# JJKK1313/DiTreeOnlinePlanner

Measured on AMD Instinct MI355X. Metric: candidate tree-expansions/sec (carmaze, H=32), higher is better.
Workload: dtype f16x3; 1 GPU; cfgs/carmaze.yaml + fm_policy flow sampler (K=1), batch=1024 candidates per GPU, H=32 (4 chunks x 8 steps), boxes.csv 20x20, 1024-node tree snapshot, seeded random weights; batch_per_gpu=1024, global_batch=1024, edge_length=32, action_horizon=8, pred_horizon=64, flow_steps=1, tree_nodes=1024, parallelism=candidates sharded x1

## Files before the change

ditreeonlineplanner_amd/csrc/conv_tiles.hip:

```cpp
#include <type_traits>

#include "denoise_device.h"

static thread_local bool g_dn_dry_run = false;
void denoise_set_dry_run(bool on) { g_dn_dry_run = on; }
bool denoise_dry_run() { return g_dn_dry_run; }

template <int PREC>
__device__ __forceinline__ void gemm_epilogue(const ConvGemmParams& p, f32x16_t (&acc)[2][4], char* smem, int tm, int tn,
                                              int tid, int lane, int r5, int h, int wm, int wn,
                                              long long out_extra_bytes = 0) {

  constexpr int ET = PREC == 2 ? 1 : 0;
  float satm = 0.0f;
  const int c_l = wn * 128 + 4 * r5;
  const int n0 = tn * 256 + c_l;
  const bool n_ok = n0 < p.N;
  float bias4[4] = {0.f, 0.f, 0.f, 0.f};
  if (p.bias != nullptr && n_ok) {
    f32x4_t t = *(const f32x4_t*)(p.bias + n0);
#pragma unroll
    for (int j = 0; j < 4; ++j) bias4[j] = t[j];
  }
#pragma unroll
  for (int mb = 0; mb < 2; ++mb)
#pragma unroll
    for (int j = 0; j < 4; ++j)
#pragma unroll
      for (int i = 0; i < 16; ++i) {
        if constexpr (PREC == 2) acc[mb][j][i] = fmaf(acc[mb][j][i], p.w_scale, bias4[j]);
        else acc[mb][j][i] += bias4[j];
      }

  int blk_b[4], blk_l[4];
#pragma unroll
  for (int blk = 0; blk < 4; ++blk) {
    const int m0 = tm * 256 + wm * 64 + (blk >> 1) * 32 + (blk & 1) * 16;
    const int b = m0 / p.L;
    blk_b[blk] = b;
    blk_l[blk] = m0 - b * p.L;
  }

  if (p.mode >= MODE_GN_MISH) {
    float* s_sum = (float*)smem;
    float* s_sq = s_sum + 64;
    if (tid < 128) s_sum[tid] = 0.0f;
    const f32x4_t gam = *(const f32x4_t*)(p.gamma + n0);
    const f32x4_t bet = *(const f32x4_t*)(p.beta + n0);
    f32x4_t film_s[4], film_b[4];
    if (p.mode == MODE_GN_MISH_FILM) {
#pragma unroll
      for (int blk = 0; blk < 4; ++blk) {
        const float* fr = p.film + (long long)blk_b[blk] * p.film_ld + p.film_off + n0;
        film_s[blk] = *(const f32x4_t*)fr;
        film_b[blk] = *(const f32x4_t*)(fr + p.N);
      }
    }
    short4_t resv[2][8];
    auto fetch_res = [&](int blk, short4_t (&dst)[8]) {
#pragma unroll
      for (int i = 0; i < 8; ++i) {
        const int rofs = (i & 3) + 8 * (i >> 2) + 4 * h;
        const long long rrow = (long long)blk_b[blk] * p.res_Lp + blk_l[blk] + rofs + p.res_off;
        dst[i] = *(const short4_t*)((const char*)p.Res + (rrow * p.ldres + n0) * 2);
      }
    };
    const bool res_bf16 = (PREC != 1) && p.mode == MODE_GN_MISH_RES;
    if (res_bf16) fetch_res(0, resv[0]);
    __syncthreads();
    const int spt = 256 / p.L;
    const int gi = c_l / p.group_ch;
    const bool wide = p.group_ch >= 128;
    int slot[4];
#pragma unroll
    for (int blk = 0; blk < 4; ++blk) slot[blk] = blk_b[blk] - tm * spt;
    const float inv_cnt = 1.0f / (float)(p.group_ch * p.L);
    const bool ordered = p.L >= 128 || (p.group_ch == 256 && p.L >= 32);
    const bool adder = lane == 0 || (!wide && lane == 16);
    const int ocell = ((wm * 2 + wn) * 4 + gi) * 2;
    auto put = [&](float* cell, float (&t)[4]) {
      if (ordered) {
        if (p.L >= 64) { t[0] = (t[0] + t[1]) + (t[2] + t[3]); t[2] = 0.0f; }
        else { t[0] += t[1]; t[2] += t[3]; }
        if (adder) { cell[ocell] = t[0]; cell[ocell + 1] = t[2]; }
      } else if (adder) {
#pragma unroll
        for (int blk = 0; blk < 4; ++blk) atomicAdd(&cell[slot[blk] * 4 + gi], t[blk]);
      }
    };
    auto get = [&](const float* cell, float (&t)[4]) {
      if (!ordered) {
#pragma unroll
        for (int blk = 0; blk < 4; ++blk) t[blk] = cell[slot[blk] * 4 + gi];
        return;
      }
#pragma unroll
      for (int blk = 0; blk < 4; blk += 2) {
        const int r0 = slot[blk] * p.L;
        const int w0 = r0 >> 6, nw = p.L >= 64 ? p.L >> 6 : 1, sub = (r0 >> 5) & 1;
        float v = 0.0f;
        for (int w = w0; w < w0 + nw; ++w) {
          v += cell[((w * 2 + 0) * 4 + gi) * 2 + sub];
          v += cell[((w * 2 + 1) * 4 + gi) * 2 + sub];
        }
        t[blk] = v; t[blk + 1] = v;
      }
    };
    float mean[4], rstd[4];
    if constexpr (PREC != 1) {
      float ps[4], pq[4];
#pragma unroll
      for (int blk = 0; blk < 4; ++blk) {
        float s = 0.f, q = 0.f;
#pragma unroll
        for (int j = 0; j < 4; ++j)
#pragma unroll
          for (int i = 0; i < 8; ++i) {
            const float v = acc[blk >> 1][j][(blk & 1) * 8 + i];
            s += v;
            q = fmaf(v, v, q);
          }
        s += __shfl_xor(s, 1); q += __shfl_xor(q, 1);
        s += __shfl_xor(s, 2); q += __shfl_xor(q, 2);
        s += __shfl_xor(s, 4); q += __shfl_xor(q, 4);
        s += __shfl_xor(s, 8); q += __shfl_xor(q, 8);
        s += __shfl_xor(s, 32); q += __shfl_xor(q, 32);
        if (wide) { s += __shfl_xor(s, 16); q += __shfl_xor(q, 16); }
        ps[blk] = s; pq[blk] = q;
      }
      put(s_sum, ps);
      put(s_sq, pq);
      __syncthreads();
      get(s_sum, ps);
      get(s_sq, pq);
#pragma unroll
      for (int blk = 0; blk < 4; ++blk) {
        mean[blk] = ps[blk] * inv_cnt;
        const float var = fmaxf(pq[blk] * inv_cnt - mean[blk] * mean[blk], 0.0f);
        rstd[blk] = rsqrtf(var + p.eps);
      }
    } else {
    {
      float ps[4];
#pragma unroll
      for (int blk = 0; blk < 4; ++blk) {
        float s = 0.f;
#pragma unroll
        for (int j = 0; j < 4; ++j)
#pragma unroll
          for (int i = 0; i < 8; ++i) s += acc[blk >> 1][j][(blk & 1) * 8 + i];
        ps[blk] = s;
      }
#pragma unroll
      for (int blk = 0; blk < 4; ++blk) {
        float s = ps[blk];
        s += __shfl_xor(s, 1); s += __shfl_xor(s, 2); s += __shfl_xor(s, 4); s += __shfl_xor(s, 8);
        s += __shfl_xor(s, 32);
        if (wide) s += __shfl_xor(s, 16);
        ps[blk] = s;
      }
      put(s_sum, ps);
      __syncthreads();
      get(s_sum, ps);
#pragma unroll
      for (int blk = 0; blk < 4; ++blk) mean[blk] = ps[blk] * inv_cnt;
    }
    {
      float ps[4];
#pragma unroll
      for (int blk = 0; blk < 4; ++blk) {
        float s = 0.f;
#pragma unroll
        for (int j = 0; j < 4; ++j)
#pragma unroll
          for (int i = 0; i < 8; ++i) {
            float d = acc[blk >> 1][j][(blk & 1) * 8 + i] - mean[blk];
            s += d * d;
          }
        s += __shfl_xor(s, 1); s += __shfl_xor(s, 2); s += __shfl_xor(s, 4); s += __shfl_xor(s, 8);
        s += __shfl_xor(s, 32);
        if (wide) s += __shfl_xor(s, 16);
        ps[blk] = s;
      }
      put(s_sq, ps);
      __syncthreads();
      get(s_sq, ps);
#pragma unroll
      for (int blk = 0; blk < 4; ++blk) rstd[blk] = rsqrtf(ps[blk] * inv_cnt + p.eps);
    }

    }

#pragma unroll
    for (int blk = 0; blk < 4; ++blk) {
      if (res_bf16 && blk < 3) fetch_res(blk + 1, resv[(blk + 1) & 1]);
      f32x4_t fs = {1.f, 1.f, 1.f, 1.f}, fb = {0.f, 0.f, 0.f, 0.f};
      if (p.mode == MODE_GN_MISH_FILM) { fs = film_s[blk]; fb = film_b[blk]; }
      float ga[4], be[4];
#pragma unroll
      for (int j = 0; j < 4; ++j) { ga[j] = gam[j] * rstd[blk]; be[j] = bet[j] - mean[blk] * ga[j]; }
#pragma unroll
      for (int i = 0; i < 8; ++i) {
        const int ii = (blk & 1) * 8 + i;
        const int rofs = (i & 3) + 8 * (i >> 2) + 4 * h;
        const int b = blk_b[blk], l = blk_l[blk] + rofs;
        float v[4];
#pragma unroll
        for (int j = 0; j < 4; ++j) v[j] = mish_f<PREC == 1 ? 1 : 0>(acc[blk >> 1][j][ii] * ga[j] + be[j]) * fs[j] + fb[j];
        if (p.mode == MODE_GN_MISH_RES) {
          if constexpr (PREC != 1) {
            const short4_t rv = resv[blk & 1][i];
#pragma unroll
            for (int j = 0; j < 4; ++j) v[j] += e2f<ET>((unsigned short)rv[j]);
          } else {
            const long long rrow = (long long)b * p.res_Lp + l + p.res_off;
            const f32x4_t rv = *(const f32x4_t*)((const char*)p.Res + (rrow * p.ldres + n0) * 4);
#pragma unroll
            for (int j = 0; j < 4; ++j) v[j] += rv[j];
          }
        }
        const long long orow = (long long)b * p.out_Lp + (long long)l * p.out_stride + p.out_off;
        const long long oidx = orow * p.ldc + p.out_coff + n0;
        if constexpr (PREC == 1) {
          const f32x4_t o = {v[0], v[1], v[2], v[3]};
          *(f32x4_t*)((char*)p.Out + out_extra_bytes + oidx * 4) = o;
        } else {
          short4_t o;
          if constexpr (ET == 1) { sat_see2(satm, v[0], v[1]); sat_see2(satm, v[2], v[3]); }
#pragma unroll
          for (int j = 0; j < 4; ++j) o[j] = (short)f2e<ET>(v[j]);
          *(short4_t*)((char*)p.Out + out_extra_bytes + oidx * 2) = o;
        }
      }
    }
    if constexpr (ET == 1) sat_flush(p.sat, satm);
    return;
  }

#pragma unroll
  for (int blk = 0; blk < 4; ++blk) {
#pragma unroll
    for (int i = 0; i < 8; ++i) {
      const int ii = (blk & 1) * 8 + i;
      const int rofs = (i & 3) + 8 * (i >> 2) + 4 * h;
      const int m = tm * 256 + wm * 64 + (blk >> 1) * 32 + (blk & 1) * 16 + rofs;
      if (m >= p.M || !n_ok) continue;
      int b = blk_b[blk], l = blk_l[blk] + rofs;
      if ((p.L & 15) != 0) { b = m / p.L; l = m - b * p.L; }
      const long long orow = (long long)b * p.out_Lp + (long long)l * p.out_stride + p.out_off;
      const long long oidx = orow * p.ldc + p.out_coff + n0;
      if (p.out_f32 || PREC == 1) {
        const f32x4_t o = {acc[blk >> 1][0][ii], acc[blk >> 1][1][ii], acc[blk >> 1][2][ii], acc[blk >> 1][3][ii]};
        *(f32x4_t*)((char*)p.Out + out_extra_bytes + oidx * 4) = o;
      } else {
        short4_t o;
        if constexpr (ET == 1) { sat_see2(satm, acc[blk >> 1][0][ii], acc[blk >> 1][1][ii]); sat_see2(satm, acc[blk >> 1][2][ii], acc[blk >> 1][3][ii]); }
#pragma unroll
        for (int j = 0; j < 4; ++j) o[j] = (short)f2e<ET>(acc[blk >> 1][j][ii]);
        *(short4_t*)((char*)p.Out + out_extra_bytes + oidx * 2) = o;
      }
    }
  }
  if constexpr (ET == 1) sat_flush(p.sat, satm);
}

template <int PREC, bool C2D = false>
__global__ void __launch_bounds__(512, 2) conv_gemm_kernel(ConvGemmParams p) {
  constexpr int ES = (PREC == 1) ? 4 : 2;
  constexpr int ET = PREC == 2 ? 1 : 0;
  constexpr int EK = 128 / ES;
  constexpr int EPS = 16 / ES;
  extern __shared__ __attribute__((aligned(16))) char smem[];

  const int tid = threadIdx.x, lane = tid & 63, w = tid >> 6;
  const int r5 = lane & 31, h = lane >> 5;
  const int wm = w >> 1, wn = w & 1;
  const int ntn = (p.N + 255) >> 8;
  const int ntm = (p.M + 255) >> 8;
  const int tile = xcd_remap(blockIdx.x, ntm * ntn);
  const int tm = tile / ntn, tn = tile - tm * ntn;
  const int K = p.taps * p.Cin;
  const int kpt = p.Cin / EK;
  int nk = K / EK;
  int k_first = 0;
  long long out_extra = 0;
  if constexpr (C2D) {
    if (p.splitk > 1) {
      const int per = (nk + p.splitk - 1) / p.splitk;
      k_first = blockIdx.y * per;
      nk = min(nk - k_first, per);
      out_extra = (long long)blockIdx.y * p.slab_stride * 4;
    }
  }

  const char* Abase = (const char*)p.A;
  const char* Wbase = (const char*)p.W;
  long long aoff[4], boff[4];
#pragma unroll
  for (int q = 0; q < 4; ++q) {
    const int r = (w * 4 + q) * 8 + (lane >> 3);
    const int sw = (r >> 1) & 7;
    const int slot = (lane & 7) ^ sw;
    int m = tm * 256 + r;
    m = m < p.M ? m : p.M - 1;
    const int b = m / p.L, l = m - b * p.L;
    aoff[q] = (((long long)b * p.in_Lp + (long long)l * p.in_stride + p.in_off) * p.lda + slot * EPS) * ES;
    const int c = (r & 128) + 4 * (r & 31) + ((r >> 5) & 3);
    boff[q] = (((long long)(tn * 256 + c)) * K + slot * EPS) * ES;
  }
  const char* pa[4];
  const char* pb[4];
#pragma unroll
  for (int q = 0; q < 4; ++q) {
    pa[q] = Abase + aoff[q];
    pb[q] = Wbase + boff[q] + (long long)k_first * 128;
  }
  int kin = C2D ? (k_first % kpt) : 0;
  const long long a_tap_jump = ((long long)p.lda - (long long)p.Cin + EK) * ES;
  const char* c2_base[4];
  int c2_ih0[4], c2_iw0[4], c2_slot[4];
  int c2_tap = C2D ? (k_first / kpt) : 0;
  if constexpr (C2D) {
#pragma unroll
    for (int q = 0; q < 4; ++q) {
      const int r = (w * 4 + q) * 8 + (lane >> 3);
      int m = tm * 256 + r;
      m = m < p.M ? m : p.M - 1;
      const int b = m / p.c2_OHW, rem = m - b * p.c2_OHW;
      const int oh = rem / p.c2_OW, ow = rem - oh * p.c2_OW;
      c2_base[q] = Abase + (long long)b * p.c2_H * p.c2_W * p.Cin * ES;
      c2_ih0[q] = oh * p.c2_stride - p.c2_pad;
      c2_iw0[q] = ow * p.c2_stride - p.c2_pad;
      c2_slot[q] = ((lane & 7) ^ ((r >> 1) & 7)) * 16;
    }
  }
  auto c2_point = [&]() {
    const int kh = p.c2_kh[c2_tap], kw = p.c2_kw[c2_tap];
#pragma unroll
    for (int q = 0; q < 4; ++q) {
      const int ih = c2_ih0[q] + kh, iw = c2_iw0[q] + kw;
      const bool ok = ih >= 0 && ih < p.c2_H && iw >= 0 && iw < p.c2_W;
      const char* src = c2_base[q] + ((long long)(ih * p.c2_W + iw) * p.Cin + kin * EK) * ES;
      pa[q] = (ok ? src : (const char*)p.zero) + c2_slot[q];
    }
  };
  if constexpr (C2D) c2_point();
  auto advance = [&]() {
    ++kin;
    if constexpr (C2D) {
      if (kin == kpt) { kin = 0; ++c2_tap; }
      if (c2_tap < p.taps) c2_point();
#pragma unroll
      for (int q = 0; q < 4; ++q) pb[q] += 128;
    } else {
      long long ainc = 128;
      if (kin == kpt) { kin = 0; ainc = a_tap_jump; }
#pragma unroll
      for (int q = 0; q < 4; ++q) {
        pa[q] += ainc;
        pb[q] += 128;
      }
    }
  };
  auto stage_piece = [&](int q, char* sbase) {
    if (q < 4)
      __builtin_amdgcn_global_load_lds((const GLOBAL_AS void*)pa[q], (LDS_AS void*)(sbase + (w * 4 + q) * 1024), 16, 0, 0);
    else
      __builtin_amdgcn_global_load_lds((const GLOBAL_AS void*)pb[q - 4],
                                       (LDS_AS void*)(sbase + 32768 + (w * 4 + q - 4) * 1024), 16, 0, 0);
  };

  f32x16_t acc[2][4];
#pragma unroll
  for (int mb = 0; mb < 2; ++mb)
#pragma unroll
    for (int j = 0; j < 4; ++j)
#pragma unroll
      for (int i = 0; i < 16; ++i) acc[mb][j][i] = 0.0f;

  const int swl = (r5 >> 1) & 7;
  const int a_row_off = (wm * 64 + r5) * 128;
  const int b_row_off = 32768 + (wn * 128 + r5) * 128;

  auto kstep = [&](const char* sb, auto stage_tag, char* snext) {
    constexpr bool STAGE = decltype(stage_tag)::value;
    if constexpr (PREC != 1) {
      short8_t af[2][2], bfr[2][4];
      auto rd = [&](int ks, int slot) {
        const int ps = (((ks << 1) | h) ^ swl) << 4;
#pragma unroll
        for (int mb = 0; mb < 2; ++mb)
          af[slot][mb] = *(const short8_t*)(sb + a_row_off + mb * 4096 + ps);
#pragma unroll
        for (int j = 0; j < 4; ++j)
          bfr[slot][j] = *(const short8_t*)(sb + b_row_off + j * 4096 + ps);
      };
      if constexpr (STAGE) {
#pragma unroll
        for (int q = 0; q < 8; ++q) stage_piece(q, snext);
      }
      rd(0, 0);
#pragma unroll
      for (int ks = 0; ks < 4; ++ks) {
        if (ks < 3) rd(ks + 1, (ks + 1) & 1);
#pragma unroll
        for (int mb = 0; mb < 2; ++mb)
#pragma unroll
          for (int j = 0; j < 4; ++j)
            acc[mb][j] = mfma32<ET>(af[ks & 1][mb], bfr[ks & 1][j], acc[mb][j]);
      }
      if constexpr (STAGE) __builtin_amdgcn_sched_group_barrier(0x020, 8, 0);
      __builtin_amdgcn_sched_group_barrier(0x100, 6, 0);
#pragma unroll
      for (int ks = 0; ks < 4; ++ks) {
        if (ks < 3) __builtin_amdgcn_sched_group_barrier(0x100, 6, 0);
        __builtin_amdgcn_sched_group_barrier(0x008, 8, 0);
      }
    } else {
#pragma unroll
      for (int sl = 0; sl < 8; ++sl) {
        const int ps = (sl ^ swl) << 4;
        f32x4_t af[2], bfr[4];
#pragma unroll
        for (int mb = 0; mb < 2; ++mb) af[mb] = *(const f32x4_t*)(sb + a_row_off + mb * 4096 + ps);
#pragma unroll
        for (int j = 0; j < 4; ++j) bfr[j] = *(const f32x4_t*)(sb + b_row_off + j * 4096 + ps);
#pragma unroll
        for (int s2 = 0; s2 < 2; ++s2) {
#pragma unroll
          for (int mb = 0; mb < 2; ++mb) {
            const float a = h ? af[mb][2 * s2 + 1] : af[mb][2 * s2];
#pragma unroll
            for (int j = 0; j < 4; ++j) {
              const float bv = h ? bfr[j][2 * s2 + 1] : bfr[j][2 * s2];
              acc[mb][j] = __builtin_amdgcn_mfma_f32_32x32x2f32(a, bv, acc[mb][j], 0, 0, 0);
            }
          }
        }
        if constexpr (STAGE) stage_piece(sl, snext);
      }
    }
  };

#pragma unroll
  for (int q = 0; q < 8; ++q) stage_piece(q, smem);
  advance();
  for (int kt = 0; kt < nk - 1; ++kt) {
    asm volatile("s_waitcnt vmcnt(0)" ::: "memory");
    __syncthreads();
    kstep(smem + (kt & 1) * 65536, std::true_type{}, smem + ((kt + 1) & 1) * 65536);
    advance();
  }
  asm volatile("s_waitcnt vmcnt(0)" ::: "memory");
  __syncthreads();
  kstep(smem + ((nk - 1) & 1) * 65536, std::false_type{}, nullptr);
  __syncthreads();
  gemm_epilogue<PREC>(p, acc, smem, tm, tn, tid, lane, r5, h, wm, wn, out_extra);
}

template <int ET, bool SPLIT, bool SHORT = false>
__device__ __forceinline__ void gemm_epilogue16(const ConvGemmParams& p, f32x4_t (&acc)[4][8], char* smem, int tm, int tn,
                                                int tid, int lane, int r4, int h4, int wm, int wn) {
  const int c_l = wn * 128 + 8 * r4;
  const int n0 = tn * 256 + c_l;
  {
    f32x4_t b0 = {0.f, 0.f, 0.f, 0.f}, b1 = b0;
    if (p.bias != nullptr) { b0 = *(const f32x4_t*)(p.bias + n0); b1 = *(const f32x4_t*)(p.bias + n0 + 4); }
    if constexpr (ET == 1) {
      const float ws = p.w_scale;
#pragma unroll
      for (int mb = 0; mb < 4; ++mb)
#pragma unroll
        for (int j = 0; j < 4; ++j) { acc[mb][j] = acc[mb][j] * ws + b0[j]; acc[mb][4 + j] = acc[mb][4 + j] * ws + b1[j]; }
    } else if (p.bias != nullptr) {
#pragma unroll
      for (int mb = 0; mb < 4; ++mb)
#pragma unroll
        for (int j = 0; j < 4; ++j) { acc[mb][j] += b0[j]; acc[mb][4 + j] += b1[j]; }
    }
  }
  constexpr bool short_l = SHORT;
  const int lane_b = short_l ? (4 * h4) / p.L : 0, lane_l = -lane_b * p.L;
  int blk_b[4], blk_l[4];
#pragma unroll
  for (int mb = 0; mb < 4; ++mb) {
    const int m0 = tm * 256 + wm * 64 + mb * 16;
    const int b = m0 / p.L;
    blk_b[mb] = b;
    blk_l[mb] = m0 - b * p.L;
  }
  auto store_row = [&](char* o, const float (&v)[8]) {
    short8_t hi, lo;
    if constexpr (ET == 1) {
      sat_check_row(p.sat, v);
#pragma unroll
      for (int jj = 0; jj < 4; ++jj) {
        const f32x2_t c = {__builtin_amdgcn_fmed3f(v[2 * jj], -65504.0f, 65504.0f),
                           __builtin_amdgcn_fmed3f(v[2 * jj + 1], -65504.0f, 65504.0f)};
        const half2_t h = __builtin_convertvector(c, half2_t);
        const short2_t hs = __builtin_bit_cast(short2_t, h);
        hi[2 * jj] = hs[0]; hi[2 * jj + 1] = hs[1];
        if constexpr (SPLIT) {
          const half2_t l = __builtin_convertvector(c - __builtin_convertvector(h, f32x2_t), half2_t);
          const short2_t ls = __builtin_bit_cast(short2_t, l);
          lo[2 * jj] = ls[0]; lo[2 * jj + 1] = ls[1];
        }
      }
    } else {
#pragma unroll
      for (int j = 0; j < 8; ++j) {
        hi[j] = (short)f2bf(v[j]);
        if constexpr (SPLIT) lo[j] = (short)f2bf(v[j] - bf2f((unsigned short)hi[j]));
      }
    }
    *(short8_t*)o = hi;
    if constexpr (SPLIT) *(short8_t*)(o + p.out_plane) = lo;
  };
  auto out_ptr = [&](int mb, int esize) {
    const long long orow = (long long)(blk_b[mb] + lane_b) * p.out_Lp + (long long)(blk_l[mb] + 4 * h4 + lane_l) * p.out_stride + p.out_off;
    return (char*)p.Out + (orow * p.ldc + p.out_coff + n0) * esize;
  };
  if (p.mode < MODE_GN_MISH) {
    const int esize = p.out_f32 ? 4 : 2;
    const long long ostep = (long long)p.out_stride * p.ldc * esize;
#pragma unroll
    for (int mb = 0; mb < 4; ++mb) {
      char* ob = out_ptr(mb, esize);
#pragma unroll
      for (int i = 0; i < 4; ++i, ob += ostep) {
        float v[8];
#pragma unroll
        for (int j = 0; j < 8; ++j) v[j] = acc[mb][j][i];
        if (p.out_f32) {
          *(f32x4_t*)ob = f32x4_t{v[0], v[1], v[2], v[3]};
          *(f32x4_t*)(ob + 16) = f32x4_t{v[4], v[5], v[6], v[7]};
        } else {
          store_row(ob, v);
        }
      }
    }
    return;
  }
  const bool has_film = p.mode == MODE_GN_MISH_FILM, has_res = p.mode == MODE_GN_MISH_RES;
  const int spt = 256 / p.L;
  const int ns = spt > 16 ? spt * 4 : 64;
  float* s_sum = (float*)smem;
  float* s_sq = s_sum + ns;
  float* s_gb = s_sq + ns;
  float* s_film = s_gb + 512;
  const bool film_direct = has_film && short_l;
  const int b_last = p.M / p.L - 1;
  for (int i = tid; i < 2 * ns; i += 512) s_sum[i] = 0.0f;
  s_gb[tid] = tid < 256 ? p.gamma[tn * 256 + tid] : p.beta[tn * 256 + tid - 256];
  if (has_film && !film_direct) {
    for (int idx = tid; idx < spt * 128; idx += 512) {
      const int sm = idx >> 7, c4 = idx & 127;
      const int b = min(tm * spt + sm, b_last);
      const float* src = p.film + (long long)b * p.film_ld + p.film_off + tn * 256 + (c4 & 63) * 4 + (c4 >> 6) * p.N;
      *(f32x4_t*)(s_film + sm * 512 + c4 * 4) = *(const f32x4_t*)src;
    }
  }
  f32x4_t rh[2], rl[2];
  const long long rstep = (long long)p.ldres * 2;
  auto fetch_film = [&](int mb) {
    const float* fr = p.film + (long long)min(blk_b[mb] + lane_b, b_last) * p.film_ld + p.film_off + n0;
    rh[0] = *(const f32x4_t*)fr; rh[1] = *(const f32x4_t*)(fr + 4);
    rl[0] = *(const f32x4_t*)(fr + p.N); rl[1] = *(const f32x4_t*)(fr + p.N + 4);
  };
  if (film_direct) fetch_film(0);
  auto fetch_res = [&](int r) {
    const long long rrow = (long long)(blk_b[r >> 2] + lane_b) * p.res_Lp + blk_l[r >> 2] + 4 * h4 + lane_l + p.res_off;
    const char* rp = (const char*)p.Res + (rrow * p.ldres + n0) * 2 + (r & 3) * rstep;
    rh[r & 1] = *(const f32x4_t*)rp;
    if constexpr (SPLIT) rl[r & 1] = *(const f32x4_t*)(rp + p.res_plane);
  };
  if (has_res) { fetch_res(0); fetch_res(1); }
  __syncthreads();
  const int gi = c_l / p.group_ch;
  const bool wide = p.group_ch >= 128;
  const float inv_cnt = 1.0f / (float)(p.group_ch * p.L);
  int slot[4];
#pragma unroll
  for (int mb = 0; mb < 4; ++mb) slot[mb] = (blk_b[mb] + lane_b - tm * spt) * 4 + gi;
  const bool ordered = !short_l && (p.L >= 128 || (p.group_ch == 256 && p.L >= 32));
  const int hsame = short_l ? (p.L == 8 ? 2 : 1) : 4;
  const bool adder = (r4 == 0 || (!wide && r4 == 8)) && (h4 & (hsame - 1)) == 0;
  const int ocell = ((wm * 2 + wn) * 4 + gi) * 2;
  auto block_sums = [&](float (&s)[4], float* cell) {
#pragma unroll
    for (int mb = 0; mb < 4; ++mb) s[mb] = dpp_add<0xB1>(s[mb]);
#pragma unroll
    for (int mb = 0; mb < 4; ++mb) s[mb] = dpp_add<0x4E>(s[mb]);
#pragma unroll
    for (int mb = 0; mb < 4; ++mb) s[mb] = dpp_add<0x141>(s[mb]);
    if (wide) {
#pragma unroll
      for (int mb = 0; mb < 4; ++mb) s[mb] = dpp_add<0x140>(s[mb]);
    }
    if (hsame >= 2) {
#pragma unroll
      for (int mb = 0; mb < 4; ++mb) s[mb] += __shfl_xor(s[mb], 16);
    }
    if (hsame == 4) {
#pragma unroll
      for (int mb = 0; mb < 4; ++mb) s[mb] += __shfl_xor(s[mb], 32);
    }
    if (ordered) {
      if (p.L >= 64) { s[0] = (s[0] + s[1]) + (s[2] + s[3]); s[2] = 0.0f; }
      else { s[0] += s[1]; s[2] += s[3]; }
      if (adder) { cell[ocell] = s[0]; cell[ocell + 1] = s[2]; }
    } else if (adder) {
#pragma unroll
      for (int mb = 0; mb < 4; ++mb) atomicAdd(&cell[slot[mb]], s[mb]);
    }
  };
  auto cell_sums = [&](const float* cell, float (&t)[4]) {
    if (!ordered) {
#pragma unroll
      for (int mb = 0; mb < 4; ++mb) t[mb] = cell[slot[mb]];
      return;
    }
#pragma unroll
    for (int mb = 0; mb < 4; mb += 2) {
      const int r0 = (blk_b[mb] - tm * spt) * p.L;
      const int w0 = r0 >> 6, nw = p.L >= 64 ? p.L >> 6 : 1, sub = (r0 >> 5) & 1;
      float v = 0.0f;
      for (int w = w0; w < w0 + nw; ++w) {
        v += cell[((w * 2 + 0) * 4 + gi) * 2 + sub];
        v += cell[((w * 2 + 1) * 4 + gi) * 2 + sub];
      }
      t[mb] = v; t[mb + 1] = v;
    }
  };
  float mean_[4], rstd_[4];
  auto pair = [&](int mb, int j, int ip) { return f32x2_t{acc[mb][j][2 * ip], acc[mb][j][2 * ip + 1]}; };
  if constexpr (!SPLIT) {
    float s[4], q[4];
#pragma unroll
    for (int mb = 0; mb < 4; ++mb) {
      f32x2_t s2 = {0.f, 0.f}, q2 = {0.f, 0.f};
#pragma unroll
      for (int j = 0; j < 8; ++j)
#pragma unroll
        for (int ip = 0; ip < 2; ++ip) {
          const f32x2_t v = pair(mb, j, ip);
          s2 += v;
          q2 = __builtin_elementwise_fma(v, v, q2);
        }
      s[mb] = s2[0] + s2[1];
      q[mb] = q2[0] + q2[1];
    }
    block_sums(s, s_sum);
    block_sums(q, s_sq);
    __syncthreads();
    cell_sums(s_sum, s);
    cell_sums(s_sq, q);
#pragma unroll
    for (int mb = 0; mb < 4; ++mb) {
      mean_[mb] = s[mb] * inv_cnt;
      const float var = fmaxf(q[mb] * inv_cnt - mean_[mb] * mean_[mb], 0.0f);
      rstd_[mb] = rsqrtf(var + p.eps);
    }
  } else {
    float s[4];
#pragma unroll
    for (int mb = 0; mb < 4; ++mb) {
      f32x2_t s2 = {0.f, 0.f};
#pragma unroll
      for (int j = 0; j < 8; ++j)
#pragma unroll
        for (int ip = 0; ip < 2; ++ip) s2 += pair(mb, j, ip);
      s[mb] = s2[0] + s2[1];
    }
    block_sums(s, s_sum);
    __syncthreads();
    cell_sums(s_sum, s);
#pragma unroll
    for (int mb = 0; mb < 4; ++mb) {
      mean_[mb] = s[mb] * inv_cnt;
      f32x2_t q2 = {0.f, 0.f};
#pragma unroll
      for (int j = 0; j < 8; ++j) {
#pragma unroll
        for (int ip = 0; ip < 2; ++ip) {
          const f32x2_t d = pair(mb, j, ip) - mean_[mb];
          q2 = __builtin_elementwise_fma(d, d, q2);
        }
        if (j & 1) __builtin_amdgcn_sched_barrier(0);
      }
      s[mb] = q2[0] + q2[1];
    }
    block_sums(s, s_sq);
    __syncthreads();
    cell_sums(s_sq, s);
#pragma unroll
    for (int mb = 0; mb < 4; ++mb) rstd_[mb] = rsqrtf(s[mb] * inv_cnt + p.eps);
  }
  const long long ostep = (long long)p.out_stride * p.ldc * 2;
#pragma unroll
  for (int mb = 0; mb < 4; ++mb) {
    float mean = mean_[mb];
    const float rstd = rstd_[mb];
    if constexpr (SPLIT) asm volatile("" : "+v"(mean));
    float ga[8], be[8], fs[8], fb[8];
    {
      const f32x4_t gam0 = *(const f32x4_t*)(s_gb + c_l), gam1 = *(const f32x4_t*)(s_gb + c_l + 4);
      const f32x4_t bet0 = *(const f32x4_t*)(s_gb + 256 + c_l), bet1 = *(const f32x4_t*)(s_gb + 256 + c_l + 4);
#pragma unroll
      for (int j = 0; j < 4; ++j) {
        ga[j] = gam0[j] * rstd; ga[4 + j] = gam1[j] * rstd;
        if constexpr (SPLIT) { be[j] = bet0[j]; be[4 + j] = bet1[j]; }
        else { be[j] = bet0[j] - mean * ga[j]; be[4 + j] = bet1[j] - mean * ga[4 + j]; }
      }
    }
    if (film_direct) {
#pragma unroll
      for (int j = 0; j < 4; ++j) { fs[j] = rh[0][j]; fs[4 + j] = rh[1][j]; fb[j] = rl[0][j]; fb[4 + j] = rl[1][j]; }
      if (mb + 1 < 4) fetch_film(mb + 1);
    } else if (has_film) {
      const float* fr = s_film + (blk_b[mb] - tm * spt) * 512 + c_l;
      const f32x4_t f0 = *(const f32x4_t*)fr, f1 = *(const f32x4_t*)(fr + 4);
      const f32x4_t f2 = *(const f32x4_t*)(fr + 256), f3 = *(const f32x4_t*)(fr + 260);
#pragma unroll
      for (int j = 0; j < 4; ++j) { fs[j] = f0[j]; fs[4 + j] = f1[j]; fb[j] = f2[j]; fb[4 + j] = f3[j]; }
    }
    char* ob = out_ptr(mb, 2);
#pragma unroll
    for (int ip = 0; ip < 2; ++ip, ob += 2 * ostep) {
      const int r = mb * 4 + 2 * ip;
      f32x2_t v[8];
      if (has_res) {
        const short8_t h0 = __builtin_bit_cast(short8_t, rh[0]), h1 = __builtin_bit_cast(short8_t, rh[1]);
#pragma unroll
        for (int j = 0; j < 8; ++j) v[j] = f32x2_t{e2f<ET>((unsigned short)h0[j]), e2f<ET>((unsigned short)h1[j])};
        if constexpr (SPLIT) {
          const short8_t l0 = __builtin_bit_cast(short8_t, rl[0]), l1 = __builtin_bit_cast(short8_t, rl[1]);
#pragma unroll
          for (int j = 0; j < 8; ++j) v[j] += f32x2_t{e2f<ET>((unsigned short)l0[j]), e2f<ET>((unsigned short)l1[j])};
        }
        if (r + 2 < 16) { fetch_res(r + 2); fetch_res(r + 3); }
      } else {
#pragma unroll
        for (int j = 0; j < 8; ++j) v[j] = f32x2_t{0.f, 0.f};
      }
#pragma unroll
      for (int j = 0; j < 8; ++j) {
        f32x2_t x = pair(mb, j, ip);
        if constexpr (SPLIT) x = (x - mean) * ga[j] + be[j];
        else x = x * ga[j] + be[j];
        x = mish2<SPLIT ? 2 : 0>(x);
        v[j] += x;
      }
      if (has_film) {
#pragma unroll
        for (int j = 0; j < 8; ++j) v[j] = v[j] * fs[j] + fb[j];
      }
      float row[8];
#pragma unroll
      for (int j = 0; j < 8; ++j) row[j] = v[j][0];
      store_row(ob, row);
#pragma unroll
      for (int j = 0; j < 8; ++j) row[j] = v[j][1];
      store_row(ob + ostep, row);
      __builtin_amdgcn_sched_barrier(0);
    }
  }
}

template <int ET>
__device__ __forceinline__ void mm16_snake(f32x4_t (&acc)[4][8], const short8_t (&a)[4], const short8_t (&b)[4], int half) {
#pragma unroll
  for (int mb = 0; mb < 4; ++mb)
#pragma unroll
    for (int jj = 0; jj < 4; ++jj) {
      const int j = (mb & 1) ? 3 - jj : jj;
      acc[mb][half * 4 + j] = mfma16<ET>(a[mb], b[j], acc[mb][half * 4 + j]);
    }
}

#ifdef HALO16_STAMP
__device__ unsigned long long g_halo_stamp[8];
extern "C" int ditree_debug_halo_stamp(unsigned long long* out) {
  return (int)hipMemcpyFromSymbol(out, HIP_SYMBOL(g_halo_stamp), sizeof(g_halo_stamp));
}
__device__ unsigned int g_x3_phase[8][32];
extern "C" int ditree_debug_x3_phase(unsigned int* out) {
  return (int)hipMemcpyFromSymbol(out, HIP_SYMBOL(g_x3_phase), sizeof(g_x3_phase));
}
#define X3_STAMP_MAX 65536
__device__ unsigned long long g_x3_stamp[X3_STAMP_MAX][6];
__device__ unsigned int g_x3_count;
extern "C" int ditree_debug_x3_stamp(unsigned long long* out, unsigned int* count, int reset) {
  int rc = (int)hipMemcpyFromSymbol(count, HIP_SYMBOL(g_x3_count), 4);
  if (rc == 0 && out != nullptr) rc = (int)hipMemcpyFromSymbol(out, HIP_SYMBOL(g_x3_stamp), sizeof(unsigned long long) * 6 * X3_STAMP_MAX);
  if (rc == 0 && reset) { unsigned int z = 0; rc = (int)hipMemcpyToSymbol(HIP_SYMBOL(g_x3_count), &z, 4); }
  return rc;
}
#endif
template <int ET>
__global__ void __launch_bounds__(512, 2) conv3_halo16_kernel(ConvGemmParams p) {
  extern __shared__ __attribute__((aligned(16))) char smem[];
  constexpr int A_BUF = 40960, W_BUF = 32768, W_BASE = 2 * A_BUF;
  const int tid = threadIdx.x, lane = tid & 63;
  const int w = __builtin_amdgcn_readfirstlane(tid >> 6);
  const int r4 = lane & 15, h4 = lane >> 4;
  const int wm = w >> 1, wn = w & 1;
  const int ntn = (p.N + 255) >> 8;
  const int ntm = (p.M + 255) >> 8;
  const int tile = xcd_remap_strips(blockIdx.x, ntm, ntn, p.xcd_strips);
  const int tm = tile / ntn, tn = tile - tm * ntn;
  const int L = p.L, Lp = p.in_Lp, S = 256 / L;
  const int a_rows = S * Lp;
  const int nc = p.Cin >> 6;
  const long long K = 3LL * p.Cin;

  unsigned pa0, pa4, pb;
  const char* const a_base = (const char*)p.A + ((long long)tm * S * Lp + p.in_off) * p.lda * 2;
  const char* const w_base = (const char*)p.W + ((long long)tn * 256) * K * 2;
  const __amdgpu_buffer_rsrc_t a_rsrc = __builtin_amdgcn_make_buffer_rsrc((void*)a_base, 0, 0x7fffffff, 0x00020000);
  const __amdgpu_buffer_rsrc_t w_rsrc = __builtin_amdgcn_make_buffer_rsrc((void*)w_base, 0, 0x7fffffff, 0x00020000);
  {
    const int r = w * 8 + (lane >> 3);
    const int slot = (lane & 7) ^ (r & 7);
    pa0 = (unsigned)((r * p.lda + slot * 8) * 2);
    const int r4r = r + 256;
    const int rs = r4r < a_rows ? r4r : a_rows - 1;
    pa4 = (unsigned)((rs * p.lda + slot * 8) * 2);
  }
  const int a_piece = 64 * p.lda * 2;
  long long wq[4];
  {
    const int lr = lane >> 3;
    const int slot = (lane & 7) ^ lr;
    pb = (unsigned)(((long long)(8 * lr) * K + slot * 8) * 2);
#pragma unroll
    for (int q = 0; q < 4; ++q) {
      const int r0 = (w * 4 + q) * 8;
      const int cu = (r0 & 128) + 8 * (r0 & 8) + ((r0 >> 4) & 7);
      wq[q] = (long long)cu * K * 2;
    }
  }
  const int w_tap = p.Cin * 2;
  auto issue_a = [&](int c, int i) {
    __builtin_amdgcn_raw_ptr_buffer_load_lds(a_rsrc, (LDS_AS void*)(smem + (c & 1) * A_BUF + (w + 8 * i) * 1024), 16,
                                             i < 4 ? pa0 : pa4, c * 128 + (i < 4 ? i * a_piece : 0), 0, 0);
  };
  auto issue_w = [&](int c, int t, int q) {
    __builtin_amdgcn_raw_ptr_buffer_load_lds(w_rsrc, (LDS_AS void*)(smem + W_BASE + ((c + t) & 1) * W_BUF + (w * 4 + q) * 1024),
                                             16, pb, (int)wq[q] + c * 128 + t * w_tap, 0, 0);
  };

  int lrow0;
  {
    const int ml = wm * 64 + r4;
    const int sb = ml / L;
    lrow0 = sb * Lp + (ml - sb * L);
  }
  int lstep[4];
#pragma unroll
  for (int mb = 0; mb < 4; ++mb) lstep[mb] = 16 * mb + 2 * (((wm * 64 + 16 * mb) / L) - ((wm * 64) / L));
  const int swl = r4 & 7;
  const int b_row_off = (wn * 128 + r4) * 128;

  f32x4_t acc[4][8];
#pragma unroll
  for (int mb = 0; mb < 4; ++mb)
#pragma unroll
    for (int j = 0; j < 8; ++j) acc[mb][j] = f32x4_t{0.f, 0.f, 0.f, 0.f};

  short8_t af[2][4], bq[2][4];
  auto rdA = [&](int set, int c, int t, int ks) {
    const char* ab = smem + (c & 1) * A_BUF;
#pragma unroll
    for (int mb = 0; mb < 4; ++mb) {
      const int row = lrow0 + lstep[mb] + t;
      const int ps = (((ks << 2) | h4) ^ (row & 7)) << 4;
      af[set][mb] = *(const short8_t*)(ab + row * 128 + ps);
    }
  };
  auto rdB = [&](int set, int c, int t, int ks, int half) {
    const char* wb = smem + W_BASE + ((c + t) & 1) * W_BUF + b_row_off + half * 8192;
    const int psb = (((ks << 2) | h4) ^ swl) << 4;
#pragma unroll
    for (int jj = 0; jj < 4; ++jj) bq[set][jj] = *(const short8_t*)(wb + jj * 2048 + psb);
  };
  auto mm = [&](int aset, int bset, int half, int mb, int jj) {
    acc[mb][half * 4 + jj] = mfma16<ET>(af[aset][mb], bq[bset][jj], acc[mb][half * 4 + jj]);
  };
  auto mm16 = [&](int aset, int bset, int half) { mm16_snake<ET>(acc, af[aset], bq[bset], half); };

  auto step = [&](auto tT, auto tNext, auto tIW, auto tIA, auto tVM, int c) {
    constexpr int T = decltype(tT)::value;
    constexpr bool HAS_NEXT = decltype(tNext)::value, ISSUE_W = decltype(tIW)::value, ISSUE_A = decltype(tIA)::value;
    constexpr int VM = decltype(tVM)::value;
    constexpr int NV = ISSUE_W ? 4 : 0;
    asm volatile("" : "+v"(lrow0));
    __builtin_amdgcn_s_setprio(2);
    rdB(1, c, T, 0, 1);
    mm16(0, 0, 0);
    __builtin_amdgcn_sched_group_barrier(0x100, 4, 0);
    __builtin_amdgcn_sched_group_barrier(0x008, 16, 0);
    __builtin_amdgcn_sched_barrier(0);
    __builtin_amdgcn_s_setprio(1);
    rdA(1, c, T, 1);
    rdB(0, c, T, 1, 0);
    mm16(0, 1, 1);
    __builtin_amdgcn_sched_group_barrier(0x100, 8, 0);
    __builtin_amdgcn_sched_group_barrier(0x008, 16, 0);
    __builtin_amdgcn_sched_barrier(0);
    __builtin_amdgcn_s_setprio(0);
    rdB(1, c, T, 1, 1);
    mm16(1, 0, 0);
    if constexpr (ISSUE_A && T != 2) {
      if constexpr (T == 0) { issue_a(c + 1, 0); issue_a(c + 1, 1); issue_a(c + 1, 2); }
      else { issue_a(c + 1, 3); issue_a(c + 1, 4); }
      __builtin_amdgcn_sched_group_barrier(0x100, 4, 0);
      __builtin_amdgcn_sched_group_barrier(0x008, 4, 0);
      __builtin_amdgcn_sched_group_barrier(0x020, 1, 0);
      __builtin_amdgcn_sched_group_barrier(0x008, 4, 0);
      __builtin_amdgcn_sched_group_barrier(0x020, 1, 0);
      __builtin_amdgcn_sched_group_barrier(0x008, 4, 0);
      if constexpr (T == 0) __builtin_amdgcn_sched_group_barrier(0x020, 1, 0);
      __builtin_amdgcn_sched_group_barrier(0x008, 4, 0);
    } else {
      __builtin_amdgcn_sched_group_barrier(0x100, 4, 0);
      __builtin_amdgcn_sched_group_barrier(0x008, 16, 0);
    }
    __builtin_amdgcn_sched_barrier(0);
    if constexpr (HAS_NEXT) {
      if constexpr (VM == 0) asm volatile("s_waitcnt vmcnt(0) lgkmcnt(0)" ::: "memory");
      else if constexpr (VM == 3) asm volatile("s_waitcnt vmcnt(3) lgkmcnt(0)" ::: "memory");
      else asm volatile("s_waitcnt vmcnt(2) lgkmcnt(0)" ::: "memory");
      __builtin_amdgcn_s_barrier();
      __builtin_amdgcn_s_setprio(3);
      constexpr int T1 = (T + 1) % 3;
      rdA(0, c + (T + 1) / 3, T1, 0);
      rdB(0, c + (T + 1) / 3, T1, 0, 0);
    }
    constexpr int T2 = (T + 2) % 3;
    const int c2 = c + (T + 2) / 3;
#pragma unroll
    for (int mb = 0; mb < 4; ++mb)
#pragma unroll
      for (int jj = 0; jj < 4; ++jj) {
        mm(1, 1, 1, mb, (mb & 1) ? 3 - jj : jj);
        const int i = mb * 4 + jj;
        const int d = (i & 1) ? -1 : (i >> 1);
        if constexpr (ISSUE_W) { if (d >= 0 && d < 4) issue_w(c2, T2, d); }
      }
    if constexpr (HAS_NEXT) __builtin_amdgcn_sched_group_barrier(0x100, 8, 1);
#pragma unroll
    for (int i = 0; i < 16; ++i) {
      __builtin_amdgcn_sched_group_barrier(0x008, 1, 1);
      if (!(i & 1) && (i >> 1) < NV) __builtin_amdgcn_sched_group_barrier(0x020, 1, 1);
    }
    __builtin_amdgcn_sched_barrier(0);
  };
  using I0 = std::integral_constant<int, 0>;
  using I1 = std::integral_constant<int, 1>;
  using I2 = std::integral_constant<int, 2>;
  using I3 = std::integral_constant<int, 3>;
  using Tt = std::true_type;
  using Ff = std::false_type;

#pragma unroll
  for (int i = 0; i < 5; ++i) issue_a(0, i);
#pragma unroll
  for (int q = 0; q < 4; ++q) issue_w(0, 0, q);
  asm volatile("s_waitcnt vmcnt(0)" ::: "memory");
  __builtin_amdgcn_s_barrier();
#pragma unroll
  for (int q = 0; q < 4; ++q) issue_w(0, 1, q);
  rdA(0, 0, 0, 0);
  rdB(0, 0, 0, 0, 0);

#ifdef HALO16_STAMP
  const unsigned long long st0 = __builtin_amdgcn_s_memtime(), rt0 = __builtin_amdgcn_s_memrealtime();
#endif
  for (int c = 0; c < nc - 2; ++c) {
    step(I0{}, Tt{}, Tt{}, Tt{}, I3{}, c);
    step(I1{}, Tt{}, Tt{}, Tt{}, I2{}, c);
    step(I2{}, Tt{}, Tt{}, Tt{}, I0{}, c);
  }
#ifdef HALO16_STAMP
  if (blockIdx.x == 100 && tid == 0 && nc >= 32) {
    g_halo_stamp[0] = __builtin_amdgcn_s_memtime() - st0;
    g_halo_stamp[1] = __builtin_amdgcn_s_memrealtime() - rt0;
    g_halo_stamp[2] = (unsigned long long)(nc - 2) * 3;
  }
#endif
  {
    const int c = nc - 2;
    step(I0{}, Tt{}, Tt{}, Tt{}, I0{}, c);
    step(I1{}, Tt{}, Tt{}, Tt{}, I0{}, c);
    step(I2{}, Tt{}, Tt{}, Ff{}, I0{}, c);
  }
  {
    const int c = nc - 1;
    step(I0{}, Tt{}, Tt{}, Ff{}, I0{}, c);
    step(I1{}, Tt{}, Ff{}, Ff{}, I0{}, c);
    step(I2{}, Ff{}, Ff{}, Ff{}, I0{}, c);
  }
  __builtin_amdgcn_s_setprio(0);
  __syncthreads();
  gemm_epilogue16<ET, false>(p, acc, smem, tm, tn, tid, lane, r4, h4, wm, wn);
}

template <int ET, bool SHORT = false, bool SPLITK = false, int NP = 5>
__global__ void __launch_bounds__(512, 2) conv3_halo16x3_kernel(ConvGemmParams p) {
  extern __shared__ __attribute__((aligned(16))) char smem[];
  static_assert(NP == 5 || NP == 6, "five or six activation pieces");
  constexpr int A_BUF = NP * 8192, W_BUF = 32768, W_BASE = 2 * A_BUF;
  const int tid = threadIdx.x, lane = tid & 63;
  const int w = __builtin_amdgcn_readfirstlane(tid >> 6);
  const int r4 = lane & 15, h4 = lane >> 4;
  const int wm = w >> 1, wn = w & 1;
  const int ntn = (p.N + 255) >> 8;
  const int ntm = (p.M + 255) >> 8;
  const int tile = xcd_remap_strips(blockIdx.x, ntm, ntn, p.xcd_strips);
  const int tm = tile / ntn, tn = tile - tm * ntn;
  const int L = p.L, Lp = p.in_Lp, S = 256 / L;
  const int a_rows = S * Lp;
  const int nv_all = p.Cin >> 5;
  const int v_lo = SPLITK ? (int)blockIdx.y * (nv_all / p.splitk) : 0;
  const int nv = SPLITK ? v_lo + nv_all / p.splitk : nv_all;
  const long long w_row = p.w_row;
  const int w_step = p.w_step;
  const unsigned a_plane = (unsigned)p.a_plane, w_plane = (unsigned)p.w_plane;

  unsigned pa0, pa4, pa5 = 0, pb;
  const char* const a_base = (const char*)p.A + ((long long)tm * S * Lp + p.in_off) * p.lda * 2;
  const char* const w_base = (const char*)p.W + ((long long)tn * 256) * w_row;
  const __amdgpu_buffer_rsrc_t a_rsrc = __builtin_amdgcn_make_buffer_rsrc((void*)a_base, 0, 0x7fffffff, 0x00020000);
  const __amdgpu_buffer_rsrc_t w_rsrc = __builtin_amdgcn_make_buffer_rsrc((void*)w_base, 0, 0x7fffffff, 0x00020000);
  {
    const int r = w * 8 + (lane >> 3);
    const int slot = (lane & 7) ^ (r & 7);
    const unsigned po = (slot & 4) ? a_plane : 0u;
    pa0 = (unsigned)((r * p.lda + (slot & 3) * 8) * 2) + po;
    const int r4r = r + 256;
    const int rs = r4r < a_rows ? r4r : a_rows - 1;
    pa4 = (unsigned)((rs * p.lda + (slot & 3) * 8) * 2) + po;
    if constexpr (NP == 6) {
      const int r5r = r + 320;
      const int rs5 = r5r < a_rows ? r5r : a_rows - 1;
      pa5 = (unsigned)((rs5 * p.lda + (slot & 3) * 8) * 2) + po;
    }
  }
  const int a_piece = 64 * p.lda * 2;
  long long wq[4];
  {
    const int lr = lane >> 3;
    const int slot = (lane & 7) ^ lr;
    pb = (unsigned)((long long)(8 * lr) * w_row + (slot & 3) * 16) + ((slot & 4) ? w_plane : 0u);
#pragma unroll
    for (int q = 0; q < 4; ++q) {
      const int r0 = (w * 4 + q) * 8;
      const int cu = (r0 & 128) + 8 * (r0 & 8) + ((r0 >> 4) & 7);
      wq[q] = (long long)cu * w_row;
    }
  }
  const int w_tap = (p.Cin >> 5) * w_step;
  auto issue_a = [&](int v, int i) {
    __builtin_amdgcn_raw_ptr_buffer_load_lds(a_rsrc, (LDS_AS void*)(smem + (v & 1) * A_BUF + (w + 8 * i) * 1024), 16,
                                             i < 4 ? pa0 : (i == 4 ? pa4 : pa5), v * 64 + (i < 4 ? i * a_piece : 0), 0, 0);
  };
  auto issue_w = [&](int v, int t, int q) {
    __builtin_amdgcn_raw_ptr_buffer_load_lds(w_rsrc, (LDS_AS void*)(smem + W_BASE + ((v + t) & 1) * W_BUF + (w * 4 + q) * 1024),
                                             16, pb, (int)wq[q] + v * w_step + t * w_tap, 0, 0);
  };

  int lrow0;
  {
    const int ml = wm * 64 + r4;
    const int sb = ml / L;
    lrow0 = sb * Lp + (ml - sb * L);
  }
  int lstep[4];
#pragma unroll
  for (int mb = 0; mb < 4; ++mb) lstep[mb] = 16 * mb + 2 * (((wm * 64 + 16 * mb) / L) - ((wm * 64) / L));
  const int swl = r4 & 7;
  const int b_row_off = (wn * 128 + r4) * 128;

  f32x4_t acc[4][8];
#pragma unroll
  for (int mb = 0; mb < 4; ++mb)
#pragma unroll
    for (int j = 0; j < 8; ++j) acc[mb][j] = f32x4_t{0.f, 0.f, 0.f, 0.f};

  short8_t af[2][4], bq[2][4];
  auto rdA = [&](int set, int v, int t, int pl) {
    const char* ab = smem + (v & 1) * A_BUF;
#pragma unroll
    for (int mb = 0; mb < 4; ++mb) {
      const int row = lrow0 + lstep[mb] + t;
      const int ps = (((pl << 2) | h4) ^ (row & 7)) << 4;
      af[set][mb] = *(const short8_t*)(ab + row * 128 + ps);
    }
  };
  auto rdB = [&](int set, int v, int t, int pl, int half) {
    const char* wb = smem + W_BASE + ((v + t) & 1) * W_BUF + b_row_off + half * 8192;
    const int psb = (((pl << 2) | h4) ^ swl) << 4;
#pragma unroll
    for (int jj = 0; jj < 4; ++jj) bq[set][jj] = *(const short8_t*)(wb + jj * 2048 + psb);
  };
  auto mm = [&](int aset, int bset, int half, int mb, int jj) {
    acc[mb][half * 4 + jj] = mfma16<ET>(af[aset][mb], bq[bset][jj], acc[mb][half * 4 + jj]);
  };
  auto mm16 = [&](int aset, int bset, int half) { mm16_snake<ET>(acc, af[aset], bq[bset], half); };

#ifdef X3_PHASE_STAMP
  unsigned pst[24];
#define PSTAMP(k) do { pst[T * 8 + (k)] = (unsigned)__builtin_amdgcn_s_memtime(); __builtin_amdgcn_sched_barrier(0); } while (0)
#else
#define PSTAMP(k) do { } while (0)
#endif
  auto step = [&](auto tT, auto tNext, auto tIW, auto tIA, auto tVM, int v) {
    constexpr int T = decltype(tT)::value;
    constexpr bool HAS_NEXT = decltype(tNext)::value, ISSUE_W = decltype(tIW)::value, ISSUE_A = decltype(tIA)::value;
    constexpr int VM = decltype(tVM)::value;
    asm volatile("" : "+v"(lrow0));
    PSTAMP(0);
    __builtin_amdgcn_s_setprio(2);
    rdB(1, v, T, 1, 1);
    mm16(0, 0, 0);
    __builtin_amdgcn_sched_group_barrier(0x100, 4, 0);
    __builtin_amdgcn_sched_group_barrier(0x008, 16, 0);
    __builtin_amdgcn_sched_barrier(0);
    PSTAMP(1);
    rdB(0, v, T, 0, 0);
    rdA(1, v, T, 1);
    mm16(0, 1, 1);
    __builtin_amdgcn_sched_group_barrier(0x100, 8, 0);
    __builtin_amdgcn_sched_group_barrier(0x008, 16, 0);
    __builtin_amdgcn_sched_barrier(0);
    PSTAMP(2);
    __builtin_amdgcn_s_setprio(1);
    rdB(1, v, T, 0, 1);
    mm16(0, 0, 0);
    __builtin_amdgcn_sched_group_barrier(0x100, 4, 0);
    __builtin_amdgcn_sched_group_barrier(0x008, 16, 0);
    __builtin_amdgcn_sched_barrier(0);
    PSTAMP(3);
    mm16(1, 0, 0);
    if constexpr (ISSUE_A && T != 2) {
      if constexpr (T == 0) { issue_a(v + 1, 0); issue_a(v + 1, 1); issue_a(v + 1, 2); }
      else { issue_a(v + 1, 3); issue_a(v + 1, 4); if constexpr (NP == 6) issue_a(v + 1, 5); }
      __builtin_amdgcn_sched_group_barrier(0x008, 4, 2);
      __builtin_amdgcn_sched_group_barrier(0x020, 1, 2);
      __builtin_amdgcn_sched_group_barrier(0x008, 4, 2);
      __builtin_amdgcn_sched_group_barrier(0x020, 1, 2);
      __builtin_amdgcn_sched_group_barrier(0x008, 4, 2);
      if constexpr (T == 0 || NP == 6) __builtin_amdgcn_sched_group_barrier(0x020, 1, 2);
      __builtin_amdgcn_sched_group_barrier(0x008, 4, 2);
    }
    __builtin_amdgcn_sched_barrier(0);
    PSTAMP(4);
    __builtin_amdgcn_s_setprio(0);
    mm16(0, 1, 1);
    __builtin_amdgcn_sched_barrier(0);
    PSTAMP(5);
    if constexpr (HAS_NEXT) {
      if constexpr (VM == 0) asm volatile("s_waitcnt vmcnt(0) lgkmcnt(0)" ::: "memory");
      else if constexpr (VM == 3) asm volatile("s_waitcnt vmcnt(3) lgkmcnt(0)" ::: "memory");
      else asm volatile("s_waitcnt vmcnt(2) lgkmcnt(0)" ::: "memory");
      __builtin_amdgcn_s_barrier();
      __builtin_amdgcn_s_setprio(3);
      PSTAMP(6);
      constexpr int T1 = (T + 1) % 3;
      rdA(0, v + (T + 1) / 3, T1, 0);
      rdB(0, v + (T + 1) / 3, T1, 1, 0);
    }
    constexpr int T2 = (T + 2) % 3;
    const int v2 = v + (T + 2) / 3;
#pragma unroll
    for (int mb = 0; mb < 4; ++mb)
#pragma unroll
      for (int jj = 0; jj < 4; ++jj) {
        mm(1, 1, 1, mb, (mb & 1) ? 3 - jj : jj);
        const int i = mb * 4 + jj;
        const int d = (i & 1) ? -1 : (i >> 1);
        if constexpr (ISSUE_W) { if (d >= 0 && d < 4) issue_w(v2, T2, d); }
      }
    if constexpr (HAS_NEXT) __builtin_amdgcn_sched_group_barrier(0x100, 8, 1);
    constexpr int NV = ISSUE_W ? 4 : 0;
#pragma unroll
    for (int i = 0; i < 16; ++i) {
      __builtin_amdgcn_sched_group_barrier(0x008, 1, 1);
      if (!(i & 1) && (i >> 1) < NV) __builtin_amdgcn_sched_group_barrier(0x020, 1, 1);
    }
    __builtin_amdgcn_sched_barrier(0);
    PSTAMP(7);
  };
#undef PSTAMP
  using I0 = std::integral_constant<int, 0>;
  using I1 = std::integral_constant<int, 1>;
  using I2 = std::integral_constant<int, 2>;
  using I3 = std::integral_constant<int, 3>;
  using Tt = std::true_type;
  using Ff = std::false_type;

#ifdef HALO16_STAMP
  const unsigned long long xs0 = __builtin_amdgcn_s_memrealtime();
#endif
#pragma unroll
  for (int i = 0; i < NP; ++i) issue_a(v_lo, i);
#pragma unroll
  for (int q = 0; q < 4; ++q) issue_w(v_lo, 0, q);
  asm volatile("s_waitcnt vmcnt(0)" ::: "memory");
  __builtin_amdgcn_s_barrier();
#pragma unroll
  for (int q = 0; q < 4; ++q) issue_w(v_lo, 1, q);
  rdA(0, v_lo, 0, 0);
  rdB(0, v_lo, 0, 1, 0);
#ifdef HALO16_STAMP
  const unsigned long long xs1 = __builtin_amdgcn_s_memrealtime();
#endif

  using IT1 = std::integral_constant<int, NP == 6 ? 3 : 2>;
  for (int v = v_lo; v < nv - 2; ++v) {
    step(I0{}, Tt{}, Tt{}, Tt{}, I3{}, v);
    step(I1{}, Tt{}, Tt{}, Tt{}, IT1{}, v);
    step(I2{}, Tt{}, Tt{}, Tt{}, I0{}, v);
  }
#ifdef X3_PHASE_STAMP
  if (blockIdx.x == 100 && lane == 0 && nv == 64) {
#pragma unroll
    for (int k = 0; k < 24; ++k) g_x3_phase[w][k] = pst[k];
    g_x3_phase[w][24] = (unsigned)nv;
  }
#endif
  {
    const int v = nv - 2;
    step(I0{}, Tt{}, Tt{}, Tt{}, I0{}, v);
    step(I1{}, Tt{}, Tt{}, Tt{}, I0{}, v);
    step(I2{}, Tt{}, Tt{}, Ff{}, I0{}, v);
  }
  {
    const int v = nv - 1;
    step(I0{}, Tt{}, Tt{}, Ff{}, I0{}, v);
    step(I1{}, Tt{}, Ff{}, Ff{}, I0{}, v);
    step(I2{}, Ff{}, Ff{}, Ff{}, I0{}, v);
  }
  __builtin_amdgcn_s_setprio(0);
  __syncthreads();
#ifdef HALO16_STAMP
  const unsigned long long xs2 = __builtin_amdgcn_s_memrealtime();
#endif
  if constexpr (SPLITK) {
    const int ntiles = ntm * ntn;
    float* mine = p.sk_ws + ((size_t)blockIdx.y * ntiles + tile) * 65536;
#pragma unroll
    for (int mb = 0; mb < 4; ++mb)
#pragma unroll
      for (int j = 0; j < 8; ++j) *(f32x4_t*)(mine + ((mb * 8 + j) * 512 + tid) * 4) = acc[mb][j];
    __threadfence();
    __syncthreads();
    int* s_last = (int*)smem;
    if (tid == 0) *s_last = atomicAdd(p.sk_cnt + tile, 1) == p.splitk - 1;
    __syncthreads();
    const bool last = *s_last != 0;
    __syncthreads();
    if (!last) return;
    __threadfence();
#pragma unroll
    for (int mb = 0; mb < 4; ++mb)
#pragma unroll
      for (int j = 0; j < 8; ++j) acc[mb][j] = f32x4_t{0.f, 0.f, 0.f, 0.f};
    for (int sp = 0; sp < p.splitk; ++sp) {
      const float* sl = p.sk_ws + ((size_t)sp * ntiles + tile) * 65536;
#pragma unroll
      for (int mb = 0; mb < 4; ++mb)
#pragma unroll
        for (int j = 0; j < 8; ++j) acc[mb][j] += *(const f32x4_t*)(sl + ((mb * 8 + j) * 512 + tid) * 4);
    }
    if (tid == 0) p.sk_cnt[tile] = 0;
  }
  gemm_epilogue16<ET, true, SHORT>(p, acc, smem, tm, tn, tid, lane, r4, h4, wm, wn);
#ifdef HALO16_STAMP
  __syncthreads();
  if (tid == 0) {
    const unsigned long long xs3 = __builtin_amdgcn_s_memrealtime();
    const unsigned int k = atomicAdd(&g_x3_count, 1u);
    if (k < X3_STAMP_MAX) {
      g_x3_stamp[k][0] = xs0; g_x3_stamp[k][1] = xs1; g_x3_stamp[k][2] = xs2; g_x3_stamp[k][3] = xs3;
      g_x3_stamp[k][4] = ((unsigned long long)nv << 32) | blockIdx.x;
      g_x3_stamp[k][5] = ((unsigned long long)__builtin_amdgcn_s_getreg((31 << 11) | 20) << 32) |
                         (unsigned int)__builtin_amdgcn_s_getreg((31 << 11) | 4);
    }
  }
#endif
}

template <int ET, bool SPLIT>
__global__ void __launch_bounds__(256) conv2d_small_kernel(ConvGemmParams p) {
  extern __shared__ __attribute__((aligned(16))) char smem[];
  constexpr int STAGE = 16384;
  constexpr int CK = SPLIT ? 32 : 64;
  const int tid = threadIdx.x, lane = tid & 63;
  const int w = __builtin_amdgcn_readfirstlane(tid >> 6);
  const int r5 = lane & 31, h = lane >> 5;
  const int wm = w >> 1, wn = w & 1;
  const int ntn = p.N >> 6;
  const int tm = blockIdx.x / ntn, tn = blockIdx.x - tm * ntn;
  const int kpt = p.Cin / CK;
  const long long K = (long long)p.taps * p.Cin;
  int k0 = 0, nk = p.taps * kpt;
  long long out_extra = 0;
  if (p.splitk > 1) {
    const int per = (nk + p.splitk - 1) / p.splitk;
    k0 = blockIdx.y * per;
    nk = min(nk - k0, per);
    out_extra = (long long)blockIdx.y * p.slab_stride;
  }

  const char* a_base[2];
  int ih0[2], iw0[2];
  const char* w_src[2];
  int slot_b[2];
  long long plane_a[2];
#pragma unroll
  for (int q = 0; q < 2; ++q) {
    const int r = (2 * w + q) * 8 + (lane >> 3);
    const int slot = (lane & 7) ^ ((r >> 1) & 7);
    slot_b[q] = SPLIT ? (slot & 3) * 16 : slot * 16;
    plane_a[q] = (SPLIT && (slot & 4)) ? p.a_plane : 0;
    const long long plane_w = (SPLIT && (slot & 4)) ? p.w_plane : 0;
    int m = tm * 64 + r;
    m = m < p.M ? m : p.M - 1;
    const int b = m / p.c2_OHW, rem = m - b * p.c2_OHW;
    const int oh = rem / p.c2_OW, ow = rem - oh * p.c2_OW;
    a_base[q] = (const char*)p.A + (long long)b * p.c2_H * p.c2_W * p.Cin * 2;
    ih0[q] = oh * p.c2_stride - p.c2_pad;
    iw0[q] = ow * p.c2_stride - p.c2_pad;
    w_src[q] = (const char*)p.W + (long long)(tn * 64 + r) * (SPLIT ? (long long)p.w_row : K * 2) + slot_b[q] + plane_w;
  }
  auto issue = [&](int kl) {
    const int k = k0 + kl;
    const int tap = k / kpt, kin = k - tap * kpt;
    const int kh = p.c2_kh[tap], kw = p.c2_kw[tap];
    char* st = smem + (kl % 3) * STAGE;
#pragma unroll
    for (int q = 0; q < 2; ++q) {
      const int ih = ih0[q] + kh, iw = iw0[q] + kw;
      const bool ok = ih >= 0 && ih < p.c2_H && iw >= 0 && iw < p.c2_W;
      const char* src = ok ? a_base[q] + ((long long)(ih * p.c2_W + iw) * p.Cin + kin * CK) * 2 + plane_a[q] : (const char*)p.zero;
      __builtin_amdgcn_global_load_lds((const GLOBAL_AS void*)(src + slot_b[q]), (LDS_AS void*)(st + (2 * w + q) * 1024), 16, 0, 0);
    }
#pragma unroll
    for (int q = 0; q < 2; ++q)
      __builtin_amdgcn_global_load_lds((const GLOBAL_AS void*)(w_src[q] + (long long)k * (SPLIT ? p.w_step : 128)),
                                       (LDS_AS void*)(st + 8192 + (2 * w + q) * 1024), 16, 0, 0);
  };

  f32x16_t acc;
#pragma unroll
  for (int i = 0; i < 16; ++i) acc[i] = 0.0f;
  const int a_row = wm * 32 + r5, b_row = wn * 32 + r5;
  const int a_off = a_row * 128, b_off = 8192 + b_row * 128;
  const int sa = (a_row >> 1) & 7, sb = (b_row >> 1) & 7;

  issue(0);
  if (nk > 1) issue(1);
  for (int k = 0; k < nk; ++k) {
    if (k + 1 < nk) asm volatile("s_waitcnt vmcnt(4)" ::: "memory");
    else asm volatile("s_waitcnt vmcnt(0)" ::: "memory");
    __builtin_amdgcn_s_barrier();
    if (k + 2 < nk) issue(k + 2);
    const char* st = smem + (k % 3) * STAGE;
    if constexpr (SPLIT) {
      short8_t af[4], bf[4];
#pragma unroll
      for (int ks = 0; ks < 4; ++ks) {
        af[ks] = *(const short8_t*)(st + a_off + ((((ks << 1) | h) ^ sa) << 4));
        bf[ks] = *(const short8_t*)(st + b_off + ((((ks << 1) | h) ^ sb) << 4));
      }
#pragma unroll
      for (int kk = 0; kk < 2; ++kk) acc = mfma32<ET>(af[kk], bf[kk + 2], acc);
#pragma unroll
      for (int kk = 0; kk < 2; ++kk) acc = mfma32<ET>(af[kk], bf[kk], acc);
#pragma unroll
      for (int kk = 0; kk < 2; ++kk) acc = mfma32<ET>(af[kk + 2], bf[kk], acc);
    } else {
#pragma unroll
      for (int ks = 0; ks < 4; ++ks) {
        const short8_t af = *(const short8_t*)(st + a_off + ((((ks << 1) | h) ^ sa) << 4));
        const short8_t bf = *(const short8_t*)(st + b_off + ((((ks << 1) | h) ^ sb) << 4));
        acc = mfma32<ET>(af, bf, acc);
      }
    }
    asm volatile("s_waitcnt lgkmcnt(0)" ::: "memory");
  }

  const int n = tn * 64 + wn * 32 + r5;
  float bias = (p.bias != nullptr && k0 == 0) ? p.bias[n] : 0.0f;
#pragma unroll
  for (int i = 0; i < 16; ++i) {
    const int m = tm * 64 + wm * 32 + (i & 3) + 8 * (i >> 2) + 4 * h;
    if (m < p.M) ((float*)p.Out)[out_extra + (long long)m * p.ldc + p.out_coff + n] = (ET == 1 ? acc[i] * p.w_scale : acc[i]) + bias;
  }
}

template <int ET, bool SPLIT, bool SHORT = false>
__global__ void __launch_bounds__(512, 2) gemm16_kernel(ConvGemmParams p) {
  extern __shared__ __attribute__((aligned(16))) char smem[];
  constexpr int BUF = 32768, W_BASE = 2 * BUF;
  const int tid = threadIdx.x, lane = tid & 63;
  const int w = __builtin_amdgcn_readfirstlane(tid >> 6);
  const int r4 = lane & 15, h4 = lane >> 4;
  const int wm = w >> 1, wn = w & 1;
  const int ntn = p.N >> 8, ntm = p.M >> 8;
  const int tile = xcd_remap_strips(blockIdx.x, ntm, ntn, p.xcd_strips);
  const int tm = tile / ntn, tn = tile - tm * ntn;
  constexpr int KB = SPLIT ? 64 : 128;
  const int nc = SPLIT ? (p.Cin >> 5) : (p.Cin >> 6), nk = p.taps * nc;
  const unsigned a_plane = (unsigned)p.a_plane, w_plane = (unsigned)p.w_plane;
  const long long K = (long long)p.taps * p.Cin;

  long long a_tile0;
  {
    const int m0 = tm * 256;
    const int b0 = m0 / p.L, l0 = m0 - b0 * p.L;
    a_tile0 = (((long long)b0 * p.in_Lp + (long long)l0 * p.in_stride + p.in_off) * p.lda) * 2;
  }
  const __amdgpu_buffer_rsrc_t a_rsrc =
      __builtin_amdgcn_make_buffer_rsrc((void*)((const char*)p.A + a_tile0), 0, 0x7fffffff, 0x00020000);
  const long long w_row = SPLIT ? (long long)p.w_row : K * 2;
  const int w_step = SPLIT ? p.w_step : 128;
  const __amdgpu_buffer_rsrc_t w_rsrc =
      __builtin_amdgcn_make_buffer_rsrc((void*)((const char*)p.W + ((long long)tn * 256) * w_row), 0, 0x7fffffff, 0x00020000);
  unsigned pae, pao, pbe, pbo;
  int aq[4], wq[4];
  {
    const int lr = lane >> 3;
    const int slot0 = (lane & 7) ^ (lr >> 1), slot1 = slot0 ^ 4;
    const int lrb = lr / p.L, lro = lrb * p.in_Lp + (lr - lrb * p.L) * p.in_stride;
    if constexpr (SPLIT) {
      pae = (unsigned)((lro * p.lda + (slot0 & 3) * 8) * 2) + ((slot0 & 4) ? a_plane : 0u);
      pao = (unsigned)((lro * p.lda + (slot1 & 3) * 8) * 2) + ((slot1 & 4) ? a_plane : 0u);
      pbe = (unsigned)((long long)(8 * lr) * w_row + (slot0 & 3) * 16) + ((slot0 & 4) ? w_plane : 0u);
      pbo = (unsigned)((long long)(8 * lr) * w_row + (slot1 & 3) * 16) + ((slot1 & 4) ? w_plane : 0u);
    } else {
      pae = (unsigned)((lro * p.lda + slot0 * 8) * 2);
      pao = (unsigned)((lro * p.lda + slot1 * 8) * 2);
      pbe = (unsigned)(((long long)(8 * lr) * K + slot0 * 8) * 2);
      pbo = (unsigned)(((long long)(8 * lr) * K + slot1 * 8) * 2);
    }
#pragma unroll
    for (int q = 0; q < 4; ++q) {
      const int r0 = (w * 4 + q) * 8;
      const int m = tm * 256 + r0;
      const int b = m / p.L, l = m - b * p.L;
      aq[q] = (int)((((long long)b * p.in_Lp + (long long)l * p.in_stride + p.in_off) * p.lda) * 2 - a_tile0);
      const int cu = (r0 & 128) + 8 * (r0 & 8) + ((r0 >> 4) & 7);
      wq[q] = (int)((long long)cu * w_row);
    }
  }
  const int tap_bytes = p.lda * 2;
  auto src_off = [&](int k, int& ao, int& wo) {
    const int t = k / nc, c = k - t * nc;
    ao = t * tap_bytes + c * KB;
    wo = k * w_step;
  };
  auto issue = [&](int kv) {
    int ao, wo;
    src_off(kv, ao, wo);
    char* ab = smem + (kv & 1) * BUF;
    char* wb = smem + W_BASE + (kv & 1) * BUF;
#pragma unroll
    for (int q = 0; q < 4; ++q)
      __builtin_amdgcn_raw_ptr_buffer_load_lds(a_rsrc, (LDS_AS void*)(ab + (w * 4 + q) * 1024), 16, (q & 1) ? pao : pae,
                                               aq[q] + ao, 0, 0);
#pragma unroll
    for (int q = 0; q < 4; ++q)
      __builtin_amdgcn_raw_ptr_buffer_load_lds(w_rsrc, (LDS_AS void*)(wb + (w * 4 + q) * 1024), 16, (q & 1) ? pbo : pbe,
                                               wq[q] + wo, 0, 0);
  };

  auto issue_wq = [&](int kv, int q) {
    int ao, wo;
    src_off(kv, ao, wo);
    __builtin_amdgcn_raw_ptr_buffer_load_lds(w_rsrc, (LDS_AS void*)(smem + W_BASE + (kv & 1) * BUF + (w * 4 + q) * 1024), 16,
                                             (q & 1) ? pbo : pbe, wq[q] + wo, 0, 0);
  };
  const int a_row = wm * 64 + r4;
  const int swa = (a_row >> 1) & 7;
  const int a_off = a_row * 128, b_off = (wn * 128 + r4) * 128;
  const int swb = (r4 >> 1) & 7;

  f32x4_t acc[4][8];
#pragma unroll
  for (int mb = 0; mb < 4; ++mb)
#pragma unroll
    for (int j = 0; j < 8; ++j) acc[mb][j] = f32x4_t{0.f, 0.f, 0.f, 0.f};
  short8_t af[2][4], bq[2][4];
  auto rdA = [&](int set, int k, int ks) {
    const char* ab = smem + (k & 1) * BUF + a_off + ((((ks << 2) | h4) ^ swa) << 4);
#pragma unroll
    for (int mb = 0; mb < 4; ++mb) af[set][mb] = *(const short8_t*)(ab + mb * 2048);
  };
  auto rdB = [&](int set, int k, int ks, int half) {
    const char* wb = smem + W_BASE + (k & 1) * BUF + b_off + half * 8192 + ((((ks << 2) | h4) ^ swb) << 4);
#pragma unroll
    for (int jj = 0; jj < 4; ++jj) bq[set][jj] = *(const short8_t*)(wb + jj * 2048);
  };
  auto mm = [&](int aset, int bset, int half, int mb, int jj) {
    acc[mb][half * 4 + jj] = mfma16<ET>(af[aset][mb], bq[bset][jj], acc[mb][half * 4 + jj]);
  };
  auto mm16 = [&](int aset, int bset, int half) {
#pragma unroll
    for (int mb = 0; mb < 4; ++mb)
#pragma unroll
      for (int jj = 0; jj < 4; ++jj) mm(aset, bset, half, mb, (mb & 1) ? 3 - jj : jj);
  };
  auto step = [&](auto tNext, auto tIssue, int k) {
    constexpr bool HAS_NEXT = decltype(tNext)::value, ISSUE = decltype(tIssue)::value;
    if constexpr (SPLIT) {
      rdB(1, k, 1, 1);
      mm16(0, 0, 0);
      if constexpr (HAS_NEXT) {
        issue_wq(k + 1, 0); issue_wq(k + 1, 1);
        __builtin_amdgcn_sched_group_barrier(0x100, 4, 0);
        __builtin_amdgcn_sched_group_barrier(0x008, 4, 0);
        __builtin_amdgcn_sched_group_barrier(0x020, 1, 0);
        __builtin_amdgcn_sched_group_barrier(0x008, 4, 0);
        __builtin_amdgcn_sched_group_barrier(0x020, 1, 0);
        __builtin_amdgcn_sched_group_barrier(0x008, 8, 0);
      } else
      {
      __builtin_amdgcn_sched_group_barrier(0x100, 4, 0);
      __builtin_amdgcn_sched_group_barrier(0x008, 16, 0);
      }
      __builtin_amdgcn_sched_barrier(0);
      rdB(0, k, 0, 0);
      rdA(1, k, 1);
      mm16(0, 1, 1);
      if constexpr (HAS_NEXT) {
        issue_wq(k + 1, 2); issue_wq(k + 1, 3);
        __builtin_amdgcn_sched_group_barrier(0x100, 8, 0);
        __builtin_amdgcn_sched_group_barrier(0x008, 4, 0);
        __builtin_amdgcn_sched_group_barrier(0x020, 1, 0);
        __builtin_amdgcn_sched_group_barrier(0x008, 4, 0);
        __builtin_amdgcn_sched_group_barrier(0x020, 1, 0);
        __builtin_amdgcn_sched_group_barrier(0x008, 8, 0);
      } else
      {
      __builtin_amdgcn_sched_group_barrier(0x100, 8, 0);
      __builtin_amdgcn_sched_group_barrier(0x008, 16, 0);
      }
      __builtin_amdgcn_sched_barrier(0);
      rdB(1, k, 0, 1);
      mm16(0, 0, 0);
      __builtin_amdgcn_sched_group_barrier(0x100, 4, 0);
      __builtin_amdgcn_sched_group_barrier(0x008, 16, 0);
      __builtin_amdgcn_sched_barrier(0);
      mm16(1, 0, 0);
      __builtin_amdgcn_sched_barrier(0);
      mm16(0, 1, 1);
      __builtin_amdgcn_sched_barrier(0);
    } else {
      rdB(1, k, 0, 1);
      mm16(0, 0, 0);
      __builtin_amdgcn_sched_group_barrier(0x100, 4, 0);
      __builtin_amdgcn_sched_group_barrier(0x008, 16, 0);
      __builtin_amdgcn_sched_barrier(0);
      rdA(1, k, 1);
      rdB(0, k, 1, 0);
      mm16(0, 1, 1);
      __builtin_amdgcn_sched_group_barrier(0x100, 8, 0);
      __builtin_amdgcn_sched_group_barrier(0x008, 16, 0);
      __builtin_amdgcn_sched_barrier(0);
      rdB(1, k, 1, 1);
      mm16(1, 0, 0);
      __builtin_amdgcn_sched_group_barrier(0x100, 4, 0);
      __builtin_amdgcn_sched_group_barrier(0x008, 16, 0);
      __builtin_amdgcn_sched_barrier(0);
    }
    int ao2 = 0, wo2 = 0;
    if constexpr (ISSUE) src_off(k + 2, ao2, wo2);
    if constexpr (HAS_NEXT) {
      asm volatile("s_waitcnt vmcnt(0) lgkmcnt(0)" ::: "memory");
      __builtin_amdgcn_s_barrier();
      rdA(0, k + 1, 0);
      rdB(0, k + 1, SPLIT ? 1 : 0, 0);
    }
#pragma unroll
    for (int mb = 0; mb < 4; ++mb)
#pragma unroll
      for (int jj = 0; jj < 4; ++jj) {
        mm(1, 1, 1, mb, (mb & 1) ? 3 - jj : jj);
        if constexpr (ISSUE) {
          const int m = mb * 4 + jj, i = (m & 1) ? -1 : (m >> 1);
          if (i >= 0 && i < 4)
            __builtin_amdgcn_raw_ptr_buffer_load_lds(a_rsrc, (LDS_AS void*)(smem + (k & 1) * BUF + (w * 4 + i) * 1024), 16,
                                                     (i & 1) ? pao : pae, aq[i] + ao2, 0, 0);
          else if (!SPLIT && i >= 4 && i < 8)
            __builtin_amdgcn_raw_ptr_buffer_load_lds(w_rsrc, (LDS_AS void*)(smem + W_BASE + (k & 1) * BUF + (w * 4 + i - 4) * 1024),
                                                     16, ((i - 4) & 1) ? pbo : pbe, wq[i - 4] + wo2, 0, 0);
        }
      }
    if constexpr (HAS_NEXT) __builtin_amdgcn_sched_group_barrier(0x100, 8, 1);
#pragma unroll
    for (int i = 0; i < 16; ++i) {
      __builtin_amdgcn_sched_group_barrier(0x008, 1, 1);
      if (ISSUE && !(i & 1) && (!SPLIT || i < 8)) __builtin_amdgcn_sched_group_barrier(0x020, 1, 1);
    }
    __builtin_amdgcn_sched_barrier(0);
  };
  using Tt = std::true_type;
  using Ff = std::false_type;

  issue(0);
  asm volatile("s_waitcnt vmcnt(0)" ::: "memory");
  __builtin_amdgcn_s_barrier();
  if (nk > 1) {
    if constexpr (SPLIT) {
      int ao, wo;
      src_off(1, ao, wo);
#pragma unroll
      for (int q = 0; q < 4; ++q)
        __builtin_amdgcn_raw_ptr_buffer_load_lds(a_rsrc, (LDS_AS void*)(smem + BUF + (w * 4 + q) * 1024), 16, (q & 1) ? pao : pae,
                                                 aq[q] + ao, 0, 0);
    } else {
      issue(1);
    }
  }
  rdA(0, 0, 0);
  rdB(0, 0, SPLIT ? 1 : 0, 0);
  for (int k = 0; k < nk - 2; ++k) step(Tt{}, Tt{}, k);
  if (nk >= 2) step(Tt{}, Ff{}, nk - 2);
  step(Ff{}, Ff{}, nk - 1);
  __syncthreads();
  gemm_epilogue16<ET, SPLIT, SHORT>(p, acc, smem, tm, tn, tid, lane, r4, h4, wm, wn);
}
enum { TILE_HALO, TILE_GEMM16, TILE_C2D_SMALL, TILE_GENERIC };
enum { TV_SPLIT = 1,
       TV_SHORT = 2,
       TV_SPLITK = 4,
       TV_NP6 = 8,
       TV_C2D = 16 };
struct TileVariant {
  void (*kernel)(ConvGemmParams);
  unsigned lds_bytes;
  unsigned block;
  int family, st;
  unsigned flags;
  int kind;
};
static const TileVariant k_tiles[] = {
    {conv3_halo16_kernel<0>, 147456, 512, TILE_HALO, ST_BF16, 0, 0},
    {conv3_halo16_kernel<1>, 147456, 512, TILE_HALO, ST_F16, 0, 0},
    {conv3_halo16x3_kernel<0>, 147456, 512, TILE_HALO, ST_BF16, TV_SPLIT, 0},
    {conv3_halo16x3_kernel<1>, 147456, 512, TILE_HALO, ST_F16, TV_SPLIT, 0},
    {conv3_halo16x3_kernel<0, true>, 147456, 512, TILE_HALO, ST_BF16, TV_SPLIT | TV_SHORT, 0},
    {conv3_halo16x3_kernel<1, true>, 147456, 512, TILE_HALO, ST_F16, TV_SPLIT | TV_SHORT, 0},
    {conv3_halo16x3_kernel<0, false, true>, 147456, 512, TILE_HALO, ST_BF16, TV_SPLIT | TV_SPLITK, 0},
    {conv3_halo16x3_kernel<1, false, true>, 147456, 512, TILE_HALO, ST_F16, TV_SPLIT | TV_SPLITK, 0},
    {conv3_halo16x3_kernel<0, true, true>, 147456, 512, TILE_HALO, ST_BF16, TV_SPLIT | TV_SHORT | TV_SPLITK, 0},
    {conv3_halo16x3_kernel<1, true, true>, 147456, 512, TILE_HALO, ST_F16, TV_SPLIT | TV_SHORT | TV_SPLITK, 0},
    {conv3_halo16x3_kernel<0, true, false, 6>, 163840, 512, TILE_HALO, ST_BF16, TV_SPLIT | TV_SHORT | TV_NP6, 0},
    {conv3_halo16x3_kernel<1, true, false, 6>, 163840, 512, TILE_HALO, ST_F16, TV_SPLIT | TV_SHORT | TV_NP6, 0},
    {gemm16_kernel<0, false>, 131072, 512, TILE_GEMM16, ST_BF16, 0, 1},
    {gemm16_kernel<1, false>, 131072, 512, TILE_GEMM16, ST_F16, 0, 1},
    {gemm16_kernel<0, true>, 131072, 512, TILE_GEMM16, ST_BF16, TV_SPLIT, 1},
    {gemm16_kernel<1, true>, 131072, 512, TILE_GEMM16, ST_F16, TV_SPLIT, 1},
    {gemm16_kernel<0, false, true>, 131072, 512, TILE_GEMM16, ST_BF16, TV_SHORT, 1},
    {gemm16_kernel<1, false, true>, 131072, 512, TILE_GEMM16, ST_F16, TV_SHORT, 1},
    {gemm16_kernel<0, true, true>, 131072, 512, TILE_GEMM16, ST_BF16, TV_SPLIT | TV_SHORT, 1},
    {gemm16_kernel<1, true, true>, 131072, 512, TILE_GEMM16, ST_F16, TV_SPLIT | TV_SHORT, 1},
    {conv2d_small_kernel<0, false>, 3 * 16384, 256, TILE_C2D_SMALL, ST_BF16, TV_C2D, 2},
    {conv2d_small_kernel<1, false>, 3 * 16384, 256, TILE_C2D_SMALL, ST_F16, TV_C2D, 2},
    {conv2d_small_kernel<0, true>, 3 * 16384, 256, TILE_C2D_SMALL, ST_BF16, TV_C2D | TV_SPLIT, 2},
    {conv2d_small_kernel<1, true>, 3 * 16384, 256, TILE_C2D_SMALL, ST_F16, TV_C2D | TV_SPLIT, 2},
    {conv_gemm_kernel<0, false>, 131072, 512, TILE_GENERIC, ST_BF16, 0, 1},
    {conv_gemm_kernel<1, false>, 131072, 512, TILE_GENERIC, ST_F32, 0, 1},
    {conv_gemm_kernel<2, false>, 131072, 512, TILE_GENERIC, ST_F16, 0, 1},
    {conv_gemm_kernel<0, true>, 131072, 512, TILE_GENERIC, ST_BF16, TV_C2D, 2},
    {conv_gemm_kernel<1, true>, 131072, 512, TILE_GENERIC, ST_F32, TV_C2D, 2},
    {conv_gemm_kernel<2, true>, 131072, 512, TILE_GENERIC, ST_F16, TV_C2D, 2},
};
static const TileVariant* find_tile(int family, int st, unsigned flags) {
  for (const TileVariant& v : k_tiles)
    if (v.family == family && v.st == st && v.flags == flags) return &v;
  return nullptr;
}

static const TileVariant* pick_tile(const ConvGemmParams& p, int fmt) {
  const int st = fmt_st(fmt);
  const bool split = fmt_split(fmt);
  const unsigned fsplit = split ? TV_SPLIT : 0;
  const bool tile16 = st != ST_F32 && !p.c2d && (p.M & 255) == 0 && (p.N & 255) == 0 && (p.Cin & 63) == 0;
  const bool l_ok = p.L >= 16 || (p.L == 8 && split) || (p.L == 4 && split && p.splitk <= 1);
  if (tile16 && p.taps == 3 && p.in_stride == 1 && p.in_Lp == p.L + 2 && (256 % p.L) == 0 && l_ok && p.Cin >= 192) {
    if (!split) return find_tile(TILE_HALO, st, 0);
    const unsigned fshort = p.L <= 8 ? TV_SHORT : 0;
    if (p.splitk > 1) return find_tile(TILE_HALO, st, TV_SPLIT | fshort | TV_SPLITK);
    return find_tile(TILE_HALO, st, TV_SPLIT | fshort | (p.L == 4 ? TV_NP6 : 0));
  }
  const bool short_l = p.L == 8 || p.L == 4;
  if (tile16 && (!p.out_f32 || p.mode == MODE_BIAS) && p.taps >= 1 && p.taps <= 3 && ((p.L & 15) == 0 || short_l) && p.M > 0 &&
      (p.mode == MODE_BIAS || (256 % p.L) == 0))
    return find_tile(TILE_GEMM16, st, fsplit | ((p.L & 15) != 0 ? TV_SHORT : 0));
  if (p.c2d && conv2d_small_eligible(fmt) && (p.N & 63) == 0 && (p.Cin & 63) == 0 && p.out_f32 && p.mode == MODE_BIAS)
    return find_tile(TILE_C2D_SMALL, st, TV_C2D | fsplit);
  if (split) return nullptr;
  return find_tile(TILE_GENERIC, st, p.c2d ? TV_C2D : 0);
}
bool conv2d_small_eligible(int fmt) { return fmt_st(fmt) != ST_F32; }
int conv_gemm_kind(const ConvGemmParams& p, int fmt) {
  const TileVariant* v = pick_tile(p, fmt);
  return v != nullptr ? v->kind : (p.c2d ? 2 : 1);
}
bool conv_gemm_supported(const ConvGemmParams& p, int fmt) { return pick_tile(p, fmt) != nullptr; }

static void ensure_lds_attrs() {
  static bool done[64] = {};
  int dev = 0;
  hipGetDevice(&dev);
  if (dev < 0 || dev >= 64 || done[dev]) return;
  done[dev] = true;
  for (const TileVariant& v : k_tiles)
    if (v.lds_bytes > 65536) hipFuncSetAttribute((const void*)v.kernel, hipFuncAttributeMaxDynamicSharedMemorySize, (int)v.lds_bytes);
}

void launch_conv_gemm(const ConvGemmParams& p, int fmt, hipStream_t s) {
  ensure_lds_attrs();
  const TileVariant* v = pick_tile(p, fmt);
  if (v != nullptr && (v->flags & TV_SPLITK) &&
      (p.sk_ws == nullptr || p.sk_cnt == nullptr || ((p.Cin >> 5) % p.splitk) != 0 || (p.Cin >> 5) / p.splitk < 2))
    throw std::runtime_error("conv_gemm: split-K of the halo kernel needs its workspace and splitk | Cin / 32, >= 2 chunks each");
  if ((v == nullptr || v->family == TILE_GENERIC) && p.mode >= MODE_GN_MISH && (p.L & 15) != 0)
    throw std::runtime_error("conv_gemm: a fused GroupNorm epilogue at L = 8 / 4 exists on the gemm16 tile only (whole 256-row tiles)");
  if (v == nullptr) throw std::runtime_error("conv_gemm: a split GEMM of this shape fits no tile (conv_gemm_supported is the contract)");
  dim3 grid(((p.M + 255) >> 8) * ((p.N + 255) >> 8));
  if (v->family == TILE_C2D_SMALL) grid.x = ((p.M + 63) >> 6) * (p.N >> 6);
  if (v->flags & (TV_SPLITK | TV_C2D)) grid.y = p.splitk > 1 ? p.splitk : 1;
  DN_LAUNCH(v->kernel, grid, dim3(v->block), v->lds_bytes, s, p);
}
```

Before: 19320 candidate expansions/s.

## Specialize halo conv kernels on sequence length to precompute LDS fragment addresses

Adds L-specialized variants of the halo-tiled conv3 kernels for L = 16, 32 and 64. In these variants the per-fragment LDS row steps are compile-time constants, so the swizzled base addresses can be precomputed once and the inner loop issues ds_reads with immediate offsets. The main loop is also unrolled by two chunks so the double-buffer parity is a compile-time constant, which removes VALU address arithmetic between the MFMAs. The tile picker routes matching shapes to the new variants. The cost is more template instantiations and extra live address registers, which could raise VGPR pressure or perturb the hand-tuned schedule; a probe script for counting the loop's instruction mix is included.

```diff
diff --git a/ditreeonlineplanner_amd/csrc/conv_tiles.hip b/ditreeonlineplanner_amd/csrc/conv_tiles.hip
--- a/ditreeonlineplanner_amd/csrc/conv_tiles.hip
+++ b/ditreeonlineplanner_amd/csrc/conv_tiles.hip
@@ -777,6 +777,24 @@
       acc[mb][half * 4 + j] = mfma16<ET>(a[mb], b[j], acc[mb][half * 4 + j]);
     }
 }
+
+template <int LM>
+__device__ __forceinline__ constexpr int halo_frag_step(int mb) {
+  return LM == 16 ? 18 * mb : LM == 32 ? 16 * mb + 2 * (mb >> 1) : 16 * mb;
+}
+template <int LM>
+__device__ __forceinline__ constexpr unsigned halo_frag_keys() {
+  unsigned m = 0;
+  for (int mb = 0; mb < 4; ++mb)
+    for (int t = 0; t < 3; ++t) m |= 1u << ((halo_frag_step<LM>(mb) + t) & 7);
+  return m;
+}
+template <int LM>
+__device__ __forceinline__ void halo_frag_bases(unsigned (&abase)[8], unsigned lds0, int lrow0, int h4) {
+#pragma unroll
+  for (int k = 0; k < 8; ++k) abase[k] = LM != 0 ? lds0 + (unsigned)(lrow0 * 128 + ((h4 ^ ((lrow0 + k) & 7)) << 4)) : 0u;
+}
+__device__ __forceinline__ short8_t halo_frag_read(unsigned addr) { return *(const LDS_AS short8_t*)(size_t)addr; }
 
 #ifdef HALO16_STAMP
 __device__ unsigned long long g_halo_stamp[8];
@@ -797,9 +815,10 @@
   return rc;
 }
 #endif
-template <int ET>
-__global__ void __launch_bounds__(512, 2) conv3_halo16_kernel(ConvGemmParams p) {
-  extern __shared__ __attribute__((aligned(16))) char smem[];
+template <int ET, int LM>
+__device__ __forceinline__ void conv3_halo16_body(const ConvGemmParams& p) {
+  extern __shared__ __attribute__((aligned(128))) char smem_halo[];
+  static_assert(LM == 0 || LM == 16 || LM == 32 || LM == 64, "L at run time, or L = 16, 32, 64 (halo_frag_step)");
   constexpr int A_BUF = 40960, W_BUF = 32768, W_BASE = 2 * A_BUF;
   const int tid = threadIdx.x, lane = tid & 63;
   const int w = __builtin_amdgcn_readfirstlane(tid >> 6);
@@ -841,12 +860,12 @@
     }
   }
   const int w_tap = p.Cin * 2;
-  auto issue_a = [&](int c, int i) {
-    __builtin_amdgcn_raw_ptr_buffer_load_lds(a_rsrc, (LDS_AS void*)(smem + (c & 1) * A_BUF + (w + 8 * i) * 1024), 16,
+  auto issue_a = [&](int par, int c, int i) {
+    __builtin_amdgcn_raw_ptr_buffer_load_lds(a_rsrc, (LDS_AS void*)(smem_halo + par * A_BUF + (w + 8 * i) * 1024), 16,
                                              i < 4 ? pa0 : pa4, c * 128 + (i < 4 ? i * a_piece : 0), 0, 0);
   };
-  auto issue_w = [&](int c, int t, int q) {
-    __builtin_amdgcn_raw_ptr_buffer_load_lds(w_rsrc, (LDS_AS void*)(smem + W_BASE + ((c + t) & 1) * W_BUF + (w * 4 + q) * 1024),
+  auto issue_w = [&](int par, int c, int t, int q) {
+    __builtin_amdgcn_raw_ptr_buffer_load_lds(w_rsrc, (LDS_AS void*)(smem_halo + W_BASE + par * W_BUF + (w * 4 + q) * 1024),
                                              16, pb, (int)wq[q] + c * 128 + t * w_tap, 0, 0);
   };
 
@@ -859,8 +878,12 @@
   int lstep[4];
 #pragma unroll
   for (int mb = 0; mb < 4; ++mb) lstep[mb] = 16 * mb + 2 * (((wm * 64 + 16 * mb) / L) - ((wm * 64) / L));
-  const int swl = r4 & 7;
-  const int b_row_off = (wn * 128 + r4) * 128;
+  unsigned abase[8];
+  halo_frag_bases<LM>(abase, (unsigned)(size_t)(LDS_AS char*)smem_halo, lrow0, h4);
+  unsigned bbase[2];
+#pragma unroll
+  for (int ks = 0; ks < 2; ++ks)
+    bbase[ks] = (unsigned)(size_t)(LDS_AS char*)smem_halo + (unsigned)(W_BASE + (wn * 128 + r4) * 128 + ((((ks << 2) | h4) ^ (r4 & 7)) << 4));
 
   f32x4_t acc[4][8];
 #pragma unroll
@@ -869,51 +892,72 @@
     for (int j = 0; j < 8; ++j) acc[mb][j] = f32x4_t{0.f, 0.f, 0.f, 0.f};
 
   short8_t af[2][4], bq[2][4];
-  auto rdA = [&](int set, int c, int t, int ks) {
-    const char* ab = smem + (c & 1) * A_BUF;
+  auto rdA = [&](int set, int par, int t, int ks) {
 #pragma unroll
     for (int mb = 0; mb < 4; ++mb) {
-      const int row = lrow0 + lstep[mb] + t;
-      const int ps = (((ks << 2) | h4) ^ (row & 7)) << 4;
-      af[set][mb] = *(const short8_t*)(ab + row * 128 + ps);
-    }
-  };
-  auto rdB = [&](int set, int c, int t, int ks, int half) {
-    const char* wb = smem + W_BASE + ((c + t) & 1) * W_BUF + b_row_off + half * 8192;
-    const int psb = (((ks << 2) | h4) ^ swl) << 4;
-#pragma unroll
-    for (int jj = 0; jj < 4; ++jj) bq[set][jj] = *(const short8_t*)(wb + jj * 2048 + psb);
+      if constexpr (LM != 0) {
+        const int d = halo_frag_step<LM>(mb) + t;
+        af[set][mb] = halo_frag_read((abase[d & 7] ^ (unsigned)(ks << 6)) + (unsigned)(par * A_BUF + d * 128));
+      } else {
+        const int row = lrow0 + lstep[mb] + t;
+        const int ps = (((ks << 2) | h4) ^ (row & 7)) << 4;
+        af[set][mb] = *(const short8_t*)(smem_halo + par * A_BUF + row * 128 + ps);
+      }
+    }
+  };
+  auto rdB = [&](int set, int par, int ks, int half) {
+    if constexpr (LM != 0) {
+#pragma unroll
+      for (int jj = 0; jj < 4; ++jj) bq[set][jj] = halo_frag_read(bbase[ks] + (unsigned)(par * W_BUF + half * 8192 + jj * 2048));
+    } else {
+      const char* wb = smem_halo + W_BASE + par * W_BUF + (wn * 128 + r4) * 128 + half * 8192;
+      const int psb = (((ks << 2) | h4) ^ (r4 & 7)) << 4;
+#pragma unroll
+      for (int jj = 0; jj < 4; ++jj) bq[set][jj] = *(const short8_t*)(wb + jj * 2048 + psb);
+    }
   };
   auto mm = [&](int aset, int bset, int half, int mb, int jj) {
     acc[mb][half * 4 + jj] = mfma16<ET>(af[aset][mb], bq[bset][jj], acc[mb][half * 4 + jj]);
   };
   auto mm16 = [&](int aset, int bset, int half) { mm16_snake<ET>(acc, af[aset], bq[bset], half); };
 
-  auto step = [&](auto tT, auto tNext, auto tIW, auto tIA, auto tVM, int c) {
+  auto step = [&](auto tT, auto tNext, auto tIW, auto tIA, auto tVM, auto tPar, int c) {
     constexpr int T = decltype(tT)::value;
     constexpr bool HAS_NEXT = decltype(tNext)::value, ISSUE_W = decltype(tIW)::value, ISSUE_A = decltype(tIA)::value;
     constexpr int VM = decltype(tVM)::value;
     constexpr int NV = ISSUE_W ? 4 : 0;
-    asm volatile("" : "+v"(lrow0));
+    constexpr int PAR = decltype(tPar)::value;
+    auto par = [&](int known, int x) { return PAR >= 0 ? known : (x & 1); };
+    const int pa = par(PAR, c);
+    const int pw = par((PAR + T) & 1, c + T);
+    if constexpr (LM != 0) {
+#pragma unroll
+      for (int i = 0; i < 8; ++i)
+        if ((halo_frag_keys<LM>() >> i) & 1) asm volatile("" : "+v"(abase[i]));
+    } else {
+      asm volatile("" : "+v"(lrow0));
+    }
+    if constexpr (LM != 0) asm volatile("" : "+v"(bbase[0]), "+v"(bbase[1]));
     __builtin_amdgcn_s_setprio(2);
-    rdB(1, c, T, 0, 1);
+    rdB(1, pw, 0, 1);
     mm16(0, 0, 0);
     __builtin_amdgcn_sched_group_barrier(0x100, 4, 0);
     __builtin_amdgcn_sched_group_barrier(0x008, 16, 0);
     __builtin_amdgcn_sched_barrier(0);
     __builtin_amdgcn_s_setprio(1);
-    rdA(1, c, T, 1);
-    rdB(0, c, T, 1, 0);
+    rdA(1, pa, T, 1);
+    rdB(0, pw, 1, 0);
     mm16(0, 1, 1);
     __builtin_amdgcn_sched_group_barrier(0x100, 8, 0);
     __builtin_amdgcn_sched_group_barrier(0x008, 16, 0);
     __builtin_amdgcn_sched_barrier(0);
     __builtin_amdgcn_s_setprio(0);
-    rdB(1, c, T, 1, 1);
+    rdB(1, pw, 1, 1);
     mm16(1, 0, 0);
     if constexpr (ISSUE_A && T != 2) {
-      if constexpr (T == 0) { issue_a(c + 1, 0); issue_a(c + 1, 1); issue_a(c + 1, 2); }
-      else { issue_a(c + 1, 3); issue_a(c + 1, 4); }
+      const int pa1 = par(PAR ^ 1, c + 1);
+      if constexpr (T == 0) { issue_a(pa1, c + 1, 0); issue_a(pa1, c + 1, 1); issue_a(pa1, c + 1, 2); }
+      else { issue_a(pa1, c + 1, 3); issue_a(pa1, c + 1, 4); }
       __builtin_amdgcn_sched_group_barrier(0x100, 4, 0);
       __builtin_amdgcn_sched_group_barrier(0x008, 4, 0);
       __builtin_amdgcn_sched_group_barrier(0x020, 1, 0);
@@ -934,8 +978,9 @@
       __builtin_amdgcn_s_barrier();
       __builtin_amdgcn_s_setprio(3);
       constexpr int T1 = (T + 1) % 3;
-      rdA(0, c + (T + 1) / 3, T1, 0);
-      rdB(0, c + (T + 1) / 3, T1, 0, 0);
+      const int cn = c + (T + 1) / 3;
+      rdA(0, par(PAR ^ ((T + 1) / 3), cn), T1, 0);
+      rdB(0, par((PAR + T + 1) & 1, cn + T1), 0, 0);
     }
     constexpr int T2 = (T + 2) % 3;
     const int c2 = c + (T + 2) / 3;
@@ -946,7 +991,7 @@
         mm(1, 1, 1, mb, (mb & 1) ? 3 - jj : jj);
         const int i = mb * 4 + jj;
         const int d = (i & 1) ? -1 : (i >> 1);
-        if constexpr (ISSUE_W) { if (d >= 0 && d < 4) issue_w(c2, T2, d); }
+        if constexpr (ISSUE_W) { if (d >= 0 && d < 4) issue_w(par((PAR + T) & 1, c2 + T2), c2, T2, d); }
       }
     if constexpr (HAS_NEXT) __builtin_amdgcn_sched_group_barrier(0x100, 8, 1);
 #pragma unroll
@@ -964,23 +1009,41 @@
   using Ff = std::false_type;
 
 #pragma unroll
-  for (int i = 0; i < 5; ++i) issue_a(0, i);
-#pragma unroll
-  for (int q = 0; q < 4; ++q) issue_w(0, 0, q);
+  for (int i = 0; i < 5; ++i) issue_a(0, 0, i);
+#pragma unroll
+  for (int q = 0; q < 4; ++q) issue_w(0, 0, 0, q);
   asm volatile("s_waitcnt vmcnt(0)" ::: "memory");
   __builtin_amdgcn_s_barrier();
 #pragma unroll
-  for (int q = 0; q < 4; ++q) issue_w(0, 1, q);
+  for (int q = 0; q < 4; ++q) issue_w(1, 0, 1, q);
   rdA(0, 0, 0, 0);
-  rdB(0, 0, 0, 0, 0);
+  rdB(0, 0, 0, 0);
 
 #ifdef HALO16_STAMP
   const unsigned long long st0 = __builtin_amdgcn_s_memtime(), rt0 = __builtin_amdgcn_s_memrealtime();
 #endif
-  for (int c = 0; c < nc - 2; ++c) {
-    step(I0{}, Tt{}, Tt{}, Tt{}, I3{}, c);
-    step(I1{}, Tt{}, Tt{}, Tt{}, I2{}, c);
-    step(I2{}, Tt{}, Tt{}, Tt{}, I0{}, c);
+  using PR = std::integral_constant<int, -1>;
+  int c = 0;
+  if constexpr (LM != 0) {
+    for (; c + 1 < nc - 2; c += 2) {
+      step(I0{}, Tt{}, Tt{}, Tt{}, I3{}, I0{}, c);
+      step(I1{}, Tt{}, Tt{}, Tt{}, I2{}, I0{}, c);
+      step(I2{}, Tt{}, Tt{}, Tt{}, I0{}, I0{}, c);
+      step(I0{}, Tt{}, Tt{}, Tt{}, I3{}, I1{}, c + 1);
+      step(I1{}, Tt{}, Tt{}, Tt{}, I2{}, I1{}, c + 1);
+      step(I2{}, Tt{}, Tt{}, Tt{}, I0{}, I1{}, c + 1);
+    }
+    for (; c < nc - 2; ++c) {
+      step(I0{}, Tt{}, Tt{}, Tt{}, I0{}, PR{}, c);
+      step(I1{}, Tt{}, Tt{}, Tt{}, I0{}, PR{}, c);
+      step(I2{}, Tt{}, Tt{}, Tt{}, I0{}, PR{}, c);
+    }
+  } else {
+    for (; c < nc - 2; ++c) {
+      step(I0{}, Tt{}, Tt{}, Tt{}, I3{}, PR{}, c);
+      step(I1{}, Tt{}, Tt{}, Tt{}, I2{}, PR{}, c);
+      step(I2{}, Tt{}, Tt{}, Tt{}, I0{}, PR{}, c);
+    }
   }
 #ifdef HALO16_STAMP
   if (blockIdx.x == 100 && tid == 0 && nc >= 32) {
@@ -991,25 +1054,32 @@
 #endif
   {
     const int c = nc - 2;
-    step(I0{}, Tt{}, Tt{}, Tt{}, I0{}, c);
-    step(I1{}, Tt{}, Tt{}, Tt{}, I0{}, c);
-    step(I2{}, Tt{}, Tt{}, Ff{}, I0{}, c);
+    step(I0{}, Tt{}, Tt{}, Tt{}, I0{}, PR{}, c);
+    step(I1{}, Tt{}, Tt{}, Tt{}, I0{}, PR{}, c);
+    step(I2{}, Tt{}, Tt{}, Ff{}, I0{}, PR{}, c);
   }
   {
     const int c = nc - 1;
-    step(I0{}, Tt{}, Tt{}, Ff{}, I0{}, c);
-    step(I1{}, Tt{}, Ff{}, Ff{}, I0{}, c);
-    step(I2{}, Ff{}, Ff{}, Ff{}, I0{}, c);
+    step(I0{}, Tt{}, Tt{}, Ff{}, I0{}, PR{}, c);
+    step(I1{}, Tt{}, Ff{}, Ff{}, I0{}, PR{}, c);
+    step(I2{}, Ff{}, Ff{}, Ff{}, I0{}, PR{}, c);
   }
   __builtin_amdgcn_s_setprio(0);
   __syncthreads();
-  gemm_epilogue16<ET, false>(p, acc, smem, tm, tn, tid, lane, r4, h4, wm, wn);
+  int te = tid;
+  asm volatile("" : "+v"(te));
+  gemm_epilogue16<ET, false>(p, acc, smem_halo, tm, tn, te, te & 63, te & 15, (te & 63) >> 4, wm, wn);
 }
-
-template <int ET, bool SHORT = false, bool SPLITK = false, int NP = 5>
-__global__ void __launch_bounds__(512, 2) conv3_halo16x3_kernel(ConvGemmParams p) {
-  extern __shared__ __attribute__((aligned(16))) char smem[];
+template <int ET>
+__global__ void __launch_bounds__(512, 2) conv3_halo16_kernel(ConvGemmParams p) { conv3_halo16_body<ET, 0>(p); }
+template <int ET, int LM>
+__global__ void __launch_bounds__(512, 2) conv3_halo16_fixed_kernel(ConvGemmParams p) { conv3_halo16_body<ET, LM>(p); }
+
+template <int ET, bool SHORT, bool SPLITK, int NP, int LM>
+__device__ __forceinline__ void conv3_halo16x3_body(const ConvGemmParams& p) {
+  extern __shared__ __attribute__((aligned(128))) char smem_halo[];
   static_assert(NP == 5 || NP == 6, "five or six activation pieces");
+  static_assert(LM == 0 || (!SHORT && !SPLITK && NP == 5), "fixed fragment addresses: whole-tile, five-piece form, L >= 16");
   constexpr int A_BUF = NP * 8192, W_BUF = 32768, W_BASE = 2 * A_BUF;
   const int tid = threadIdx.x, lane = tid & 63;
   const int w = __builtin_amdgcn_readfirstlane(tid >> 6);
@@ -1061,12 +1131,12 @@
     }
   }
   const int w_tap = (p.Cin >> 5) * w_step;
-  auto issue_a = [&](int v, int i) {
-    __builtin_amdgcn_raw_ptr_buffer_load_lds(a_rsrc, (LDS_AS void*)(smem + (v & 1) * A_BUF + (w + 8 * i) * 1024), 16,
+  auto issue_a = [&](int par, int v, int i) {
+    __builtin_amdgcn_raw_ptr_buffer_load_lds(a_rsrc, (LDS_AS void*)(smem_halo + par * A_BUF + (w + 8 * i) * 1024), 16,
                                              i < 4 ? pa0 : (i == 4 ? pa4 : pa5), v * 64 + (i < 4 ? i * a_piece : 0), 0, 0);
   };
-  auto issue_w = [&](int v, int t, int q) {
-    __builtin_amdgcn_raw_ptr_buffer_load_lds(w_rsrc, (LDS_AS void*)(smem + W_BASE + ((v + t) & 1) * W_BUF + (w * 4 + q) * 1024),
+  auto issue_w = [&](int par, int v, int t, int q) {
+    __builtin_amdgcn_raw_ptr_buffer_load_lds(w_rsrc, (LDS_AS void*)(smem_halo + W_BASE + par * W_BUF + (w * 4 + q) * 1024),
                                              16, pb, (int)wq[q] + v * w_step + t * w_tap, 0, 0);
   };
 
@@ -1079,6 +1149,8 @@
   int lstep[4];
 #pragma unroll
   for (int mb = 0; mb < 4; ++mb) lstep[mb] = 16 * mb + 2 * (((wm * 64 + 16 * mb) / L) - ((wm * 64) / L));
+  unsigned abase[8];
+  halo_frag_bases<LM>(abase, (unsigned)(size_t)(LDS_AS char*)smem_halo, lrow0, h4);
   const int swl = r4 & 7;
   const int b_row_off = (wn * 128 + r4) * 128;
 
@@ -1089,17 +1161,22 @@
     for (int j = 0; j < 8; ++j) acc[mb][j] = f32x4_t{0.f, 0.f, 0.f, 0.f};
 
   short8_t af[2][4], bq[2][4];
-  auto rdA = [&](int set, int v, int t, int pl) {
-    const char* ab = smem + (v & 1) * A_BUF;
+  auto rdA = [&](int set, int par, int t, int pl) {
+    const char* ab = smem_halo + par * A_BUF;
 #pragma unroll
     for (int mb = 0; mb < 4; ++mb) {
-      const int row = lrow0 + lstep[mb] + t;
-      const int ps = (((pl << 2) | h4) ^ (row & 7)) << 4;
-      af[set][mb] = *(const short8_t*)(ab + row * 128 + ps);
-    }
-  };
-  auto rdB = [&](int set, int v, int t, int pl, int half) {
-    const char* wb = smem + W_BASE + ((v + t) & 1) * W_BUF + b_row_off + half * 8192;
+      if constexpr (LM != 0) {
+        const int d = halo_frag_step<LM>(mb) + t;
+        af[set][mb] = halo_frag_read((abase[d & 7] ^ (unsigned)(pl << 6)) + (unsigned)(par * A_BUF + d * 128));
+      } else {
+        const int row = lrow0 + lstep[mb] + t;
+        const int ps = (((pl << 2) | h4) ^ (row & 7)) << 4;
+        af[set][mb] = *(const short8_t*)(ab + row * 128 + ps);
+      }
+    }
+  };
+  auto rdB = [&](int set, int par, int pl, int half) {
+    const char* wb = smem_halo + W_BASE + par * W_BUF + b_row_off + half * 8192;
     const int psb = (((pl << 2) | h4) ^ swl) << 4;
 #pragma unroll
     for (int jj = 0; jj < 4; ++jj) bq[set][jj] = *(const short8_t*)(wb + jj * 2048 + psb);
@@ -1115,28 +1192,38 @@
 #else
 #define PSTAMP(k) do { } while (0)
 #endif
-  auto step = [&](auto tT, auto tNext, auto tIW, auto tIA, auto tVM, int v) {
+  auto step = [&](auto tT, auto tNext, auto tIW, auto tIA, auto tVM, auto tPar, int v) {
     constexpr int T = decltype(tT)::value;
     constexpr bool HAS_NEXT = decltype(tNext)::value, ISSUE_W = decltype(tIW)::value, ISSUE_A = decltype(tIA)::value;
     constexpr int VM = decltype(tVM)::value;
-    asm volatile("" : "+v"(lrow0));
+    constexpr int PAR = decltype(tPar)::value;
+    auto par = [&](int known, int x) { return PAR >= 0 ? known : (x & 1); };
+    const int pa = par(PAR, v);
+    const int pw = par((PAR + T) & 1, v + T);
+    if constexpr (LM != 0) {
+#pragma unroll
+      for (int i = 0; i < 8; ++i)
+        if ((halo_frag_keys<LM>() >> i) & 1) asm volatile("" : "+v"(abase[i]));
+    } else {
+      asm volatile("" : "+v"(lrow0));
+    }
     PSTAMP(0);
     __builtin_amdgcn_s_setprio(2);
-    rdB(1, v, T, 1, 1);
+    rdB(1, pw, 1, 1);
     mm16(0, 0, 0);
     __builtin_amdgcn_sched_group_barrier(0x100, 4, 0);
     __builtin_amdgcn_sched_group_barrier(0x008, 16, 0);
     __builtin_amdgcn_sched_barrier(0);
     PSTAMP(1);
-    rdB(0, v, T, 0, 0);
-    rdA(1, v, T, 1);
+    rdB(0, pw, 0, 0);
+    rdA(1, pa, T, 1);
     mm16(0, 1, 1);
     __builtin_amdgcn_sched_group_barrier(0x100, 8, 0);
     __builtin_amdgcn_sched_group_barrier(0x008, 16, 0);
     __builtin_amdgcn_sched_barrier(0);
     PSTAMP(2);
     __builtin_amdgcn_s_setprio(1);
-    rdB(1, v, T, 0, 1);
+    rdB(1, pw, 0, 1);
     mm16(0, 0, 0);
     __builtin_amdgcn_sched_group_barrier(0x100, 4, 0);
     __builtin_amdgcn_sched_group_barrier(0x008, 16, 0);
@@ -1144,8 +1231,9 @@
     PSTAMP(3);
     mm16(1, 0, 0);
     if constexpr (ISSUE_A && T != 2) {
-      if constexpr (T == 0) { issue_a(v + 1, 0); issue_a(v + 1, 1); issue_a(v + 1, 2); }
-      else { issue_a(v + 1, 3); issue_a(v + 1, 4); if constexpr (NP == 6) issue_a(v + 1, 5); }
+      const int pa1 = par(PAR ^ 1, v + 1);
+      if constexpr (T == 0) { issue_a(pa1, v + 1, 0); issue_a(pa1, v + 1, 1); issue_a(pa1, v + 1, 2); }
+      else { issue_a(pa1, v + 1, 3); issue_a(pa1, v + 1, 4); if constexpr (NP == 6) issue_a(pa1, v + 1, 5); }
       __builtin_amdgcn_sched_group_barrier(0x008, 4, 2);
       __builtin_amdgcn_sched_group_barrier(0x020, 1, 2);
       __builtin_amdgcn_sched_group_barrier(0x008, 4, 2);
@@ -1168,8 +1256,9 @@
       __builtin_amdgcn_s_setprio(3);
       PSTAMP(6);
       constexpr int T1 = (T + 1) % 3;
-      rdA(0, v + (T + 1) / 3, T1, 0);
-      rdB(0, v + (T + 1) / 3, T1, 1, 0);
+      const int vn = v + (T + 1) / 3;
+      rdA(0, par(PAR ^ ((T + 1) / 3), vn), T1, 0);
+      rdB(0, par((PAR + T + 1) & 1, vn + T1), 1, 0);
     }
     constexpr int T2 = (T + 2) % 3;
     const int v2 = v + (T + 2) / 3;
@@ -1180,7 +1269,7 @@
         mm(1, 1, 1, mb, (mb & 1) ? 3 - jj : jj);
         const int i = mb * 4 + jj;
         const int d = (i & 1) ? -1 : (i >> 1);
-        if constexpr (ISSUE_W) { if (d >= 0 && d < 4) issue_w(v2, T2, d); }
+        if constexpr (ISSUE_W) { if (d >= 0 && d < 4) issue_w(par((PAR + T) & 1, v2 + T2), v2, T2, d); }
       }
     if constexpr (HAS_NEXT) __builtin_amdgcn_sched_group_barrier(0x100, 8, 1);
     constexpr int NV = ISSUE_W ? 4 : 0;
@@ -1204,24 +1293,36 @@
   const unsigned long long xs0 = __builtin_amdgcn_s_memrealtime();
 #endif
 #pragma unroll
-  for (int i = 0; i < NP; ++i) issue_a(v_lo, i);
-#pragma unroll
-  for (int q = 0; q < 4; ++q) issue_w(v_lo, 0, q);
+  for (int i = 0; i < NP; ++i) issue_a(v_lo & 1, v_lo, i);
+#pragma unroll
+  for (int q = 0; q < 4; ++q) issue_w(v_lo & 1, v_lo, 0, q);
   asm volatile("s_waitcnt vmcnt(0)" ::: "memory");
   __builtin_amdgcn_s_barrier();
 #pragma unroll
-  for (int q = 0; q < 4; ++q) issue_w(v_lo, 1, q);
-  rdA(0, v_lo, 0, 0);
-  rdB(0, v_lo, 0, 1, 0);
+  for (int q = 0; q < 4; ++q) issue_w((v_lo & 1) ^ 1, v_lo, 1, q);
+  rdA(0, v_lo & 1, 0, 0);
+  rdB(0, v_lo & 1, 1, 0);
 #ifdef HALO16_STAMP
   const unsigned long long xs1 = __builtin_amdgcn_s_memrealtime();
 #endif
 
   using IT1 = std::integral_constant<int, NP == 6 ? 3 : 2>;
-  for (int v = v_lo; v < nv - 2; ++v) {
-    step(I0{}, Tt{}, Tt{}, Tt{}, I3{}, v);
-    step(I1{}, Tt{}, Tt{}, Tt{}, IT1{}, v);
-    step(I2{}, Tt{}, Tt{}, Tt{}, I0{}, v);
+  using PR = std::integral_constant<int, -1>;
+  int v = v_lo;
+  if constexpr (LM != 0) {
+    for (; v + 1 < nv - 2; v += 2) {
+      step(I0{}, Tt{}, Tt{}, Tt{}, I3{}, I0{}, v);
+      step(I1{}, Tt{}, Tt{}, Tt{}, IT1{}, I0{}, v);
+      step(I2{}, Tt{}, Tt{}, Tt{}, I0{}, I0{}, v);
+      step(I0{}, Tt{}, Tt{}, Tt{}, I3{}, I1{}, v + 1);
+      step(I1{}, Tt{}, Tt{}, Tt{}, IT1{}, I1{}, v + 1);
+      step(I2{}, Tt{}, Tt{}, Tt{}, I0{}, I1{}, v + 1);
+    }
+  }
+  for (; v < nv - 2; ++v) {
+    step(I0{}, Tt{}, Tt{}, Tt{}, I3{}, PR{}, v);
+    step(I1{}, Tt{}, Tt{}, Tt{}, IT1{}, PR{}, v);
+    step(I2{}, Tt{}, Tt{}, Tt{}, I0{}, PR{}, v);
   }
 #ifdef X3_PHASE_STAMP
   if (blockIdx.x == 100 && lane == 0 && nv == 64) {
@@ -1232,15 +1333,15 @@
 #endif
   {
     const int v = nv - 2;
-    step(I0{}, Tt{}, Tt{}, Tt{}, I0{}, v);
-    step(I1{}, Tt{}, Tt{}, Tt{}, I0{}, v);
-    step(I2{}, Tt{}, Tt{}, Ff{}, I0{}, v);
+    step(I0{}, Tt{}, Tt{}, Tt{}, I0{}, PR{}, v);
+    step(I1{}, Tt{}, Tt{}, Tt{}, I0{}, PR{}, v);
+    step(I2{}, Tt{}, Tt{}, Ff{}, I0{}, PR{}, v);
   }
   {
     const int v = nv - 1;
-    step(I0{}, Tt{}, Tt{}, Ff{}, I0{}, v);
-    step(I1{}, Tt{}, Ff{}, Ff{}, I0{}, v);
-    step(I2{}, Ff{}, Ff{}, Ff{}, I0{}, v);
+    step(I0{}, Tt{}, Tt{}, Ff{}, I0{}, PR{}, v);
+    step(I1{}, Tt{}, Ff{}, Ff{}, I0{}, PR{}, v);
+    step(I2{}, Ff{}, Ff{}, Ff{}, I0{}, PR{}, v);
   }
   __builtin_amdgcn_s_setprio(0);
   __syncthreads();
@@ -1256,7 +1357,7 @@
       for (int j = 0; j < 8; ++j) *(f32x4_t*)(mine + ((mb * 8 + j) * 512 + tid) * 4) = acc[mb][j];
     __threadfence();
     __syncthreads();
-    int* s_last = (int*)smem;
+    int* s_last = (int*)smem_halo;
     if (tid == 0) *s_last = atomicAdd(p.sk_cnt + tile, 1) == p.splitk - 1;
     __syncthreads();
     const bool last = *s_last != 0;
@@ -1276,7 +1377,7 @@
     }
     if (tid == 0) p.sk_cnt[tile] = 0;
   }
-  gemm_epilogue16<ET, true, SHORT>(p, acc, smem, tm, tn, tid, lane, r4, h4, wm, wn);
+  gemm_epilogue16<ET, true, SHORT>(p, acc, smem_halo, tm, tn, tid, lane, r4, h4, wm, wn);
 #ifdef HALO16_STAMP
   __syncthreads();
   if (tid == 0) {
@@ -1291,6 +1392,10 @@
   }
 #endif
 }
+template <int ET, bool SHORT = false, bool SPLITK = false, int NP = 5>
+__global__ void __launch_bounds__(512, 2) conv3_halo16x3_kernel(ConvGemmParams p) { conv3_halo16x3_body<ET, SHORT, SPLITK, NP, 0>(p); }
+template <int ET, int LM>
+__global__ void __launch_bounds__(512, 2) conv3_halo16x3_fixed_kernel(ConvGemmParams p) { conv3_halo16x3_body<ET, false, false, 5, LM>(p); }
 
 template <int ET, bool SPLIT>
 __global__ void __launch_bounds__(256) conv2d_small_kernel(ConvGemmParams p) {
@@ -1459,8 +1564,8 @@
   const int tap_bytes = p.lda * 2;
   auto src_off = [&](int k, int& ao, int& wo) {
     const int t = k / nc, c = k - t * nc;
-    ao = t * tap_bytes + c * KB;
-    wo = k * w_step;
+    ao = __builtin_amdgcn_readfirstlane(t * tap_bytes + c * KB);
+    wo = __builtin_amdgcn_readfirstlane(k * w_step);
   };
   auto issue = [&](int kv) {
     int ao, wo;
@@ -1638,7 +1743,8 @@
        TV_SHORT = 2,
        TV_SPLITK = 4,
        TV_NP6 = 8,
-       TV_C2D = 16 };
+       TV_C2D = 16,
+       TV_L16 = 32, TV_L32 = 64, TV_L64 = 128 };
 struct TileVariant {
   void (*kernel)(ConvGemmParams);
   unsigned lds_bytes;
@@ -1652,6 +1758,18 @@
     {conv3_halo16_kernel<1>, 147456, 512, TILE_HALO, ST_F16, 0, 0},
     {conv3_halo16x3_kernel<0>, 147456, 512, TILE_HALO, ST_BF16, TV_SPLIT, 0},
     {conv3_halo16x3_kernel<1>, 147456, 512, TILE_HALO, ST_F16, TV_SPLIT, 0},
+    {conv3_halo16_fixed_kernel<0, 16>, 147456, 512, TILE_HALO, ST_BF16, TV_L16, 0},
+    {conv3_halo16_fixed_kernel<1, 16>, 147456, 512, TILE_HALO, ST_F16, TV_L16, 0},
+    {conv3_halo16_fixed_kernel<0, 32>, 147456, 512, TILE_HALO, ST_BF16, TV_L32, 0},
+    {conv3_halo16_fixed_kernel<1, 32>, 147456, 512, TILE_HALO, ST_F16, TV_L32, 0},
+    {conv3_halo16_fixed_kernel<0, 64>, 147456, 512, TILE_HALO, ST_BF16, TV_L64, 0},
+    {conv3_halo16_fixed_kernel<1, 64>, 147456, 512, TILE_HALO, ST_F16, TV_L64, 0},
+    {conv3_halo16x3_fixed_kernel<0, 16>, 147456, 512, TILE_HALO, ST_BF16, TV_SPLIT | TV_L16, 0},
+    {conv3_halo16x3_fixed_kernel<1, 16>, 147456, 512, TILE_HALO, ST_F16, TV_SPLIT | TV_L16, 0},
+    {conv3_halo16x3_fixed_kernel<0, 32>, 147456, 512, TILE_HALO, ST_BF16, TV_SPLIT | TV_L32, 0},
+    {conv3_halo16x3_fixed_kernel<1, 32>, 147456, 512, TILE_HALO, ST_F16, TV_SPLIT | TV_L32, 0},
+    {conv3_halo16x3_fixed_kernel<0, 64>, 147456, 512, TILE_HALO, ST_BF16, TV_SPLIT | TV_L64, 0},
+    {conv3_halo16x3_fixed_kernel<1, 64>, 147456, 512, TILE_HALO, ST_F16, TV_SPLIT | TV_L64, 0},
     {conv3_halo16x3_kernel<0, true>, 147456, 512, TILE_HALO, ST_BF16, TV_SPLIT | TV_SHORT, 0},
     {conv3_halo16x3_kernel<1, true>, 147456, 512, TILE_HALO, ST_F16, TV_SPLIT | TV_SHORT, 0},
     {conv3_halo16x3_kernel<0, false, true>, 147456, 512, TILE_HALO, ST_BF16, TV_SPLIT | TV_SPLITK, 0},
@@ -1692,10 +1810,12 @@
   const bool tile16 = st != ST_F32 && !p.c2d && (p.M & 255) == 0 && (p.N & 255) == 0 && (p.Cin & 63) == 0;
   const bool l_ok = p.L >= 16 || (p.L == 8 && split) || (p.L == 4 && split && p.splitk <= 1);
   if (tile16 && p.taps == 3 && p.in_stride == 1 && p.in_Lp == p.L + 2 && (256 % p.L) == 0 && l_ok && p.Cin >= 192) {
-    if (!split) return find_tile(TILE_HALO, st, 0);
+    const unsigned flen = p.L == 64 ? TV_L64 : (p.L == 32 ? TV_L32 : (p.L == 16 ? TV_L16 : 0));
+    if (!split) return find_tile(TILE_HALO, st, flen);
     const unsigned fshort = p.L <= 8 ? TV_SHORT : 0;
     if (p.splitk > 1) return find_tile(TILE_HALO, st, TV_SPLIT | fshort | TV_SPLITK);
-    return find_tile(TILE_HALO, st, TV_SPLIT | fshort | (p.L == 4 ? TV_NP6 : 0));
+    if (p.L >= 16) return find_tile(TILE_HALO, st, TV_SPLIT | flen);
+    return find_tile(TILE_HALO, st, TV_SPLIT | TV_SHORT | (p.L == 4 ? TV_NP6 : 0));
   }
   const bool short_l = p.L == 8 || p.L == 4;
   if (tile16 && (!p.out_f32 || p.mode == MODE_BIAS) && p.taps >= 1 && p.taps <= 3 && ((p.L & 15) == 0 || short_l) && p.M > 0 &&
diff --git a/profiles/probes/loop_mix.py b/profiles/probes/loop_mix.py
--- /dev/null
+++ b/profiles/probes/loop_mix.py
@@ -0,0 +1,160 @@
+import argparse
+import os
+import re
+import shutil
+import subprocess
+import sys
+import tempfile
+
+REPO = os.path.dirname(os.path.dirname(os.path.dirname(os.path.abspath(__file__))))
+sys.path.insert(0, REPO)
+from ditreeonlineplanner_amd import build as B
+
+DEFAULT = ["conv3_halo16x3_kernel", "conv3_halo16_kernel", "gemm16_kernel", "conv2d_small_kernel"]
+
+
+def compile_asm(out, defines=()):
+    extra = dict(B.UNITS)["conv_tiles.hip"]
+    cmd = [B.HIPCC, *B.COMMON, *extra, *defines, "--cuda-device-only", "-S", os.path.join(B.CSRC, "conv_tiles.hip"), "-o", out]
+    subprocess.check_call(cmd)
+
+
+def demangle(names):
+    filt = shutil.which("llvm-cxxfilt") or shutil.which("c++filt")
+    if filt is None:
+        raise SystemExit("loop_mix: needs llvm-cxxfilt or c++filt on PATH to name the template instantiations")
+    out = subprocess.run([filt], input="\n".join(names), capture_output=True, text=True, check=True).stdout.split("\n")
+    return dict(zip(names, out))
+
+
+def kernels_of(text):
+    lines = text.split("\n")
+    syms = re.findall(r"^\s*\.amdhsa_kernel\s+(\S+)", text, re.M)
+    bodies = {}
+    start = {}
+    for i, ln in enumerate(lines):
+        m = re.match(r"^(\w+):", ln)
+        if m:
+            start.setdefault(m.group(1), i)
+    for s in syms:
+        if s not in start:
+            continue
+        a = start[s]
+        b = a
+        while b < len(lines) and not lines[b].lstrip().startswith("s_endpgm"):
+            b += 1
+        bodies[s] = lines[a + 1:b + 1]
+    meta = {}
+    cur = None
+    for ln in lines:
+        m = re.match(r"\s*-?\s*\.(\w+):\s*(.*)$", ln)
+        if not m:
+            continue
+        k, v = m.group(1), m.group(2).strip()
+        if ln.lstrip().startswith("- .") and k in ("agpr_count", "args"):
+            cur = {}
+        if cur is not None:
+            cur[k] = v
+            if k == "name" and v in bodies:
+                meta[v] = cur
+    return bodies, meta
+
+
+def insn(ln):
+    s = ln.split(";")[0].strip()
+    if not s or s.startswith(".") or s.endswith(":"):
+        return None
+    return s
+
+
+def largest_loop(body):
+    label_at = {}
+    for i, ln in enumerate(body):
+        m = re.match(r"^(\.LBB\d+_\d+):", ln)
+        if m:
+            label_at[m.group(1)] = i
+    last_back = {}
+    for i, ln in enumerate(body):
+        s = insn(ln)
+        if s and (s.startswith("s_cbranch") or s.startswith("s_branch")):
+            tgt = s.split()[-1]
+            if tgt in label_at and label_at[tgt] < i:
+                last_back[tgt] = i
+    best = None
+    for tgt, i in last_back.items():
+        ins = [s for s in map(insn, body[label_at[tgt]:i + 1]) if s]
+        key = (sum(s.startswith("v_mfma") for s in ins), len(ins))
+        if best is None or key > best[0]:
+            best = (key, label_at[tgt], i)
+    return best
+
+
+def count(lines):
+    c = dict(mfma=0, valu=0, salu=0, waitcnt=0, lds=0, lds_imm=0, buffer=0, other=0, valu_ops={}, salu_ops={})
+    for ln in lines:
+        s = insn(ln)
+        if not s:
+            continue
+        op = s.split()[0]
+        if op.startswith("v_mfma"):
+            c["mfma"] += 1
+        elif op.startswith("v_"):
+            c["valu"] += 1
+            c["valu_ops"][op] = c["valu_ops"].get(op, 0) + 1
+        elif op == "s_waitcnt":
+            c["waitcnt"] += 1
+        elif op.startswith("s_"):
+            c["salu"] += 1
+            c["salu_ops"][op] = c["salu_ops"].get(op, 0) + 1
+        elif op.startswith("ds_"):
+            c["lds"] += 1
+            c["lds_imm"] += "offset:" in s
+        elif op.startswith("buffer_"):
+            c["buffer"] += 1
+        else:
+            c["other"] += 1
+    return c
+
+
+def main():
+    ap = argparse.ArgumentParser()
+    ap.add_argument("patterns", nargs="*", help="substrings of the demangled kernel name (all given ones must match)")
+    ap.add_argument("--asm", help="count this assembly file instead of compiling")
+    ap.add_argument("--keep", help="write the assembly here")
+    ap.add_argument("-D", action="append", default=[], help="extra define for the compile (diagnostic builds)")
+    ap.add_argument("--ops", action="store_true", help="list the VALU / SALU opcodes of each loop")
+    args = ap.parse_args()
+    if args.asm:
+        path = args.asm
+    else:
+        path = args.keep or os.path.join(tempfile.mkdtemp(prefix="loop_mix_"), "conv_tiles.s")
+        compile_asm(path, ["-D" + d for d in args.D])
+    with open(path) as f:
+        bodies, meta = kernels_of(f.read())
+    names = demangle(list(bodies))
+    pats = args.patterns
+    print(f"{'kernel':<58s} {'MFMA':>5s} {'VALU':>5s} {'SALU':>5s} {'wait':>5s} {'LDS':>4s} {'+imm':>4s} {'buf':>4s} "
+          f"{'VALU/100':>8s} {'SALU/100':>8s} {'VGPR':>5s} {'spill':>5s} {'scratch':>7s}")
+    for sym in sorted(bodies, key=lambda s: names[s]):
+        nm = re.sub(r"^void |\(ConvGemmParams\)$", "", names[sym])
+        if pats and not all(p in nm for p in pats):
+            continue
+        if not pats and not any(nm.startswith(d + "<") for d in DEFAULT):
+            continue
+        lp = largest_loop(bodies[sym])
+        if lp is None:
+            print(f"{nm:<58s} (no loop)")
+            continue
+        c = count(bodies[sym][lp[1]:lp[2] + 1])
+        m = meta.get(sym, {})
+        per = 100.0 / max(c["mfma"], 1)
+        print(f"{nm:<58s} {c['mfma']:5d} {c['valu']:5d} {c['salu']:5d} {c['waitcnt']:5d} {c['lds']:4d} {c['lds_imm']:4d} "
+              f"{c['buffer']:4d} {c['valu'] * per:8.1f} {c['salu'] * per:8.1f} {m.get('vgpr_count', '?'):>5s} "
+              f"{m.get('vgpr_spill_count', '?'):>5s} {m.get('private_segment_fixed_size', '?'):>7s}")
+        if args.ops:
+            for kind in ("valu_ops", "salu_ops"):
+                print("    " + kind[:4] + ": " + ", ".join(f"{n} {k}" for k, n in sorted(c[kind].items(), key=lambda kv: -kv[1])))
+
+
+if __name__ == "__main__":
+    main()
```

New measurement: 19690 candidate expansions/s (median of 6 runs). 1.9% higher.
